# yuecideng/Misc3D

Hardware: AMD Instinct MI355X
Metric: RANSAC hypotheses/sec, 1M-pt cloud (inlier-score GB/s: roofline.algorithmic_reuse) (higher is better)
Workload: dtype f64 decisions (fp32 screen + fp64 recount)

## Files before the change

### include/misc3d_amd.h

```cpp
#ifndef MISC3D_AMD_H
#define MISC3D_AMD_H

#include <stddef.h>
#include <stdint.h>

#ifdef __cplusplus
extern "C" {
#endif

#define M3D_OK 1
#define M3D_FALSE 0
#define M3D_ERR_PROBABILITY (-1)
#define M3D_ERR_TOO_FEW_POINTS (-2)
#define M3D_ERR_NO_NORMALS (-3)
#define M3D_ERR_SIZE_MISMATCH (-4)
#define M3D_ERR_INVALID_ARG (-5)
#define M3D_ERR_DEVICE (-6)
#define M3D_ERR_INTERNAL (-7)
#define M3D_ERR_NON_FINITE (-8)

enum m3d_model_kind { M3D_PLANE = 0, M3D_SPHERE = 1, M3D_CYLINDER = 2 };

typedef struct m3d_stats {
    double fitness;
// ... 360 lines not shown
    uint64_t n_rays;
    uint64_t pair_tests;
    uint64_t nodes_visited;
} m3d_raycast_stats;
int m3d_raycast_pinhole(const m3d_raycast_mesh *meshes, size_t n_meshes, const double *poses, size_t n_poses, size_t n_frames,
                        int width, int height, double fx, double fy, double cx, double cy, int device, float *t_hit,
                        uint32_t *geometry_ids, uint32_t *primitive_ids, float *primitive_normals, m3d_raycast_stats *stats);

int m3d_match_mutual_nn(const double *feat_src, size_t n_src, const double *feat_dst, size_t n_dst,
                        int dim, int method, int n_trees, int device, size_t *out_src,
                        size_t *out_dst, size_t *k);
uint64_t m3d_match_last_fallbacks(void);

typedef struct m3d_comm m3d_comm;
#define M3D_COMM_ID_BYTES 128
int m3d_comm_unique_id(uint8_t id[M3D_COMM_ID_BYTES]);
m3d_comm *m3d_comm_create_rccl(const uint8_t id[M3D_COMM_ID_BYTES], int world, int rank, int device);
typedef int (*m3d_allgather_fn)(void *user, const void *send, void *recv, size_t bytes_per_rank);
m3d_comm *m3d_comm_create_host(int world, int rank, m3d_allgather_fn fn, void *user);
int m3d_comm_create_local(int world, m3d_comm **comms );
void m3d_comm_destroy(m3d_comm *comm);
int m3d_comm_world(const m3d_comm *comm);
int m3d_comm_rank(const m3d_comm *comm);
uint64_t m3d_comm_collectives(const m3d_comm *comm);

int m3d_cloud_fit_sharded(m3d_cloud *cloud, m3d_comm *comm, int kind, double threshold, size_t max_iteration,
                          double probability, const uint64_t *seed, double *params, size_t *inliers,
                          size_t *n_inliers, m3d_stats *stats);
int m3d_segment_plane_iterative_sharded(const double *xyz, size_t n, double threshold, int max_iteration,
                                        double min_ratio, const uint64_t *seed, int device, m3d_comm *comm,
                                        size_t max_clusters, double *planes, size_t *cluster_offsets,
                                        size_t *cluster_indices, size_t *n_clusters);
int m3d_segment_plane_iterative_multi(const double *xyz, size_t n, double threshold, int max_iteration,
                                      double min_ratio, const uint64_t *seed, const int *devices, int n_dev,
                                      size_t max_clusters, double *planes, size_t *cluster_offsets,
                                      size_t *cluster_indices, size_t *n_clusters);
int m3d_fit_multi(int kind, const double *xyz, const double *normals, size_t n, double threshold,
                  size_t max_iteration, double probability, const uint64_t *seed, const int *devices, int n_dev,
                  double *params, size_t *inliers, size_t *n_inliers, m3d_stats *stats);
int m3d_registration_ransac_sharded(const double *src, size_t n_src, const double *dst, size_t n_dst,
                                    const size_t *corr_src, const size_t *corr_dst, size_t m, double threshold,
                                    int max_iter, double edge_length_threshold, double confidence,
                                    const uint64_t *seed, int device, m3d_comm *comm, double T[16],
                                    m3d_reg_stats *stats);

typedef struct m3d_config {
    int32_t dense_scoring;
    int32_t speculative_refine;
    int32_t lead_hypotheses;
    int32_t score_groups_per_block;
    int32_t score_min_workgroups;
    int32_t dense_workgroups;
    int32_t reg_neighbour_lists;
    int32_t reg_prune;
    int32_t match_brute;
    int32_t match_fp32_screen;
    int32_t pool_limit_mb;
    int32_t kernel_timing;
    int32_t reg_sorted_lists;
    int32_t score_fp32_screen;
    int32_t cull_fp32;
    int32_t reg_fp32_screen;
    int32_t sorted_tombstones;
    int32_t score_mfma;
    int32_t score_mfma_groups;
    int32_t score_waves4;
    int32_t score_waves4_groups;
    int32_t score_phases;
    int32_t compact_one_pass;
    int32_t plane_bound;
    int32_t lanes;
    int32_t wait_spin_us;
    int32_t prestream;
    int32_t chunk_cap;
    int32_t first_chunk;
    int32_t reg_cells_per_radius;
    int32_t match_pipeline;
    int32_t reg_cache;
    int32_t device_aliases;
    int32_t lanes_eager;
    int32_t list_mask;
    int32_t mask_early;
    int32_t ref_bound;
} m3d_config;
void m3d_get_config(m3d_config *out);
int m3d_set_config(const m3d_config *in);

const char *m3d_last_error(void);
int m3d_device_count(void);
const char *m3d_version(void);

#ifdef __cplusplus
}
#endif
#endif
```

### include/misc3d_amd_bench.h

```cpp
#ifndef MISC3D_AMD_BENCH_H
#define MISC3D_AMD_BENCH_H

#include "misc3d_amd.h"

#ifdef __cplusplus
extern "C" {
#endif

int m3d_bench_time_score(m3d_cloud *cloud, int kind, double threshold, const uint32_t *samples,
                         size_t n_hypotheses, int reps, int mode, double *ms_avg,
                         uint64_t *listed_pairs);


int m3d_bench_fp64_issue_rate(int device, double ms_target, double *tera_lane_ops_per_s, double *ms_measured);

int m3d_bench_cloud_setup_ms(const m3d_cloud *cloud, double out[5]);

int m3d_bench_plane_upper_bounds(m3d_cloud *cloud, double threshold, const uint32_t *samples, size_t n_hypotheses,
                                 uint32_t *ub_out);
int m3d_bench_plane_ref_upper_bounds(m3d_cloud *cloud, double threshold, const uint32_t *samples, size_t n_hypotheses,
                                     size_t ref_index, uint32_t *ub_out);
int m3d_bench_upper_bounds(m3d_cloud *cloud, int kind, double threshold, const uint32_t *samples, size_t n_hypotheses,
                           uint32_t *ub_out);
int m3d_bench_last_segment_ms(double out[6]);

int m3d_bench_reg_checkers(const double *ps, const double *pd, const double *T, double edge_threshold,
                           double distance_threshold);

int m3d_bench_kabsch_sums(const double *src, const double *dst, size_t n, int device, double out[18]);

int m3d_bench_icp_sums(const double *src, size_t n_src, const double *dst, size_t n_dst, double max_correspondence_distance,
                       const double *T, int device, double out[29], int64_t *corr);

int m3d_bench_fps_force_path(int path);

int m3d_bench_knn_force_path(int path);

int m3d_bench_knn_tile_merge(const double *data, size_t n, int dim, const double *queries, size_t m, int kk, int pages,
                             int splits, uint32_t rows_per_split, int device, uint32_t *idx_out, uint64_t *d2_bits_out);

int m3d_bench_voxel_force_path(int path);

int m3d_bench_proximity_cutoffs(double dist, double angle_deg, double out[5]);

int m3d_bench_fpfh_pair_bins(const double *pairs, size_t m, int32_t *bins, double *features);

unsigned m3d_bench_match_last_path(void);

#ifdef __cplusplus
}
#endif
#endif
```

### misc3d_amd/capi.py

```python
from __future__ import annotations

import ctypes as C
import threading
import os
import sys
from dataclasses import dataclass

import numpy as np

_HERE = os.path.dirname(os.path.abspath(__file__))
FP_ORDER = int(os.environ.get("M3D_FP_ORDER", "0") or 0)
_VARIANT = os.environ.get("M3D_LIB_VARIANT", "")
LIB_PATH = os.path.join(_HERE, "lib", *([_VARIANT] if _VARIANT else ([f"order{FP_ORDER}"] if FP_ORDER else [])), "libmisc3d_amd.so")
HEADER_PATH = os.path.join(os.path.dirname(_HERE), "include", "misc3d_amd.h")

PLANE, SPHERE, CYLINDER = 0, 1, 2
MINIMAL_SAMPLE = {PLANE: 3, SPHERE: 4, CYLINDER: 2}
NUM_PARAMS = {PLANE: 4, SPHERE: 4, CYLINDER: 7}
MODEL_STRIDE = 8

OK, FALSE = 1, 0
ERR_PROBABILITY, ERR_TOO_FEW_POINTS, ERR_NO_NORMALS, ERR_SIZE_MISMATCH = -1, -2, -3, -4
ERR_INVALID_ARG, ERR_DEVICE, ERR_INTERNAL = -5, -6, -7
ERR_NON_FINITE = -8
# ... 152 lines not shown
        L.m3d_raycast_pinhole.argtypes = [C.c_void_p, C.c_size_t, C.c_void_p, C.c_size_t, C.c_size_t, C.c_int, C.c_int, C.c_double,
                                          C.c_double, C.c_double, C.c_double, C.c_int, C.c_void_p, C.c_void_p, C.c_void_p,
                                          C.c_void_p, C.c_void_p]
        L.m3d_proximity_segment.argtypes = [C.c_void_p, C.c_void_p, C.c_size_t, C.c_size_t, C.c_double, C.c_void_p,
                                            C.c_size_t, C.c_size_t, C.c_int, C.c_void_p, C.c_void_p, C.c_void_p, C.c_void_p,
                                            C.c_void_p]
        L.m3d_proximity_segment_nn.argtypes = [C.c_void_p, C.c_void_p, C.c_size_t, C.c_size_t, C.c_size_t, C.c_void_p,
                                               C.c_void_p, C.c_void_p, C.c_size_t, C.c_size_t, C.c_int, C.c_void_p,
                                               C.c_void_p, C.c_void_p, C.c_void_p, C.c_void_p]
        L.m3d_radius_neighbors.argtypes = [C.c_void_p, C.c_size_t, C.c_double, C.c_int, C.c_void_p, C.c_void_p, C.c_void_p,
                                           C.c_size_t, C.c_void_p]
        L.m3d_bench_proximity_cutoffs.argtypes = [C.c_double, C.c_double, C.c_void_p]
        L.m3d_knn_create.restype = C.c_void_p
        L.m3d_knn_create.argtypes = [C.c_void_p, C.c_size_t, C.c_int, C.c_int, C.c_void_p]
        L.m3d_knn_destroy.restype = None
        L.m3d_knn_destroy.argtypes = [C.c_void_p]
        L.m3d_knn_size.restype = C.c_size_t
        L.m3d_knn_size.argtypes = [C.c_void_p]
        L.m3d_knn_dim.argtypes = [C.c_void_p]
        L.m3d_knn_search.argtypes = [C.c_void_p, C.c_void_p, C.c_size_t, C.c_int, C.c_int64, C.c_double, C.c_size_t,
                                     C.c_void_p, C.c_void_p, C.c_void_p, C.c_void_p, C.c_void_p]
        L.m3d_bench_knn_force_path.argtypes = [C.c_int]
        L.m3d_bench_knn_tile_merge.argtypes = [C.c_void_p, C.c_size_t, C.c_int, C.c_void_p, C.c_size_t, C.c_int, C.c_int,
                                               C.c_int, C.c_uint32, C.c_int, C.c_void_p, C.c_void_p]
        L.m3d_estimate_normals.argtypes = [C.c_void_p, C.c_size_t, C.c_int, C.c_double, C.c_int, C.c_int, C.c_void_p, C.c_int,
                                           C.c_void_p, C.c_void_p]
        L.m3d_compute_fpfh.argtypes = [C.c_void_p, C.c_void_p, C.c_size_t, C.c_int, C.c_double, C.c_int, C.c_int, C.c_void_p,
                                       C.c_void_p]
        L.m3d_preprocess_fragment.argtypes = [C.c_void_p, C.c_void_p, C.c_size_t, C.c_double, C.c_int, C.c_void_p, C.c_void_p,
                                              C.c_void_p]
        L.m3d_bench_fpfh_pair_bins.argtypes = [C.c_void_p, C.c_size_t, C.c_void_p, C.c_void_p]
        L.m3d_match_last_fallbacks.restype = C.c_uint64
        L.m3d_match_last_fallbacks.argtypes = []
        L.m3d_match_mutual_nn.argtypes = [C.c_void_p, C.c_size_t, C.c_void_p, C.c_size_t, C.c_int, C.c_int, C.c_int,
                                          C.c_int, C.c_void_p, C.c_void_p, C.c_void_p]
        L.m3d_comm_unique_id.argtypes = [C.c_void_p]
        L.m3d_comm_create_rccl.restype = C.c_void_p
        L.m3d_comm_create_rccl.argtypes = [C.c_void_p, C.c_int, C.c_int, C.c_int]
        L.m3d_comm_create_host.restype = C.c_void_p
        L.m3d_comm_create_host.argtypes = [C.c_int, C.c_int, ALLGATHER_FN, C.c_void_p]
        L.m3d_comm_create_local.argtypes = [C.c_int, C.c_void_p]
        L.m3d_comm_destroy.restype = None
        L.m3d_comm_destroy.argtypes = [C.c_void_p]
        L.m3d_comm_world.argtypes = [C.c_void_p]
        L.m3d_comm_rank.argtypes = [C.c_void_p]
        L.m3d_comm_collectives.restype = C.c_uint64
        L.m3d_comm_collectives.argtypes = [C.c_void_p]
        L.m3d_cloud_fit_sharded.argtypes = [C.c_void_p, C.c_void_p, C.c_int, C.c_double, C.c_size_t, C.c_double, C.c_void_p,
                                            C.c_void_p, C.c_void_p, C.c_void_p, C.c_void_p]
        L.m3d_segment_plane_iterative_clouds.argtypes = [C.c_void_p, C.c_size_t, C.c_double, C.c_int, C.c_double,
                                                          C.c_void_p, C.c_int, C.c_size_t, C.c_void_p, C.c_void_p,
                                                          C.c_void_p, C.c_void_p, C.c_void_p]
        L.m3d_segment_plane_iterative_sharded.argtypes = [C.c_void_p, C.c_size_t, C.c_double, C.c_int, C.c_double,
                                                          C.c_void_p, C.c_int, C.c_void_p, C.c_size_t, C.c_void_p,
                                                          C.c_void_p, C.c_void_p, C.c_void_p]
        L.m3d_segment_plane_iterative_multi.argtypes = [C.c_void_p, C.c_size_t, C.c_double, C.c_int, C.c_double,
                                                        C.c_void_p, C.c_void_p, C.c_int, C.c_size_t, C.c_void_p,
                                                        C.c_void_p, C.c_void_p, C.c_void_p]
        L.m3d_fit_multi.argtypes = [C.c_int, C.c_void_p, C.c_void_p, C.c_size_t, C.c_double, C.c_size_t, C.c_double,
                                    C.c_void_p, C.c_void_p, C.c_int, C.c_void_p, C.c_void_p, C.c_void_p, C.c_void_p]
        L.m3d_registration_ransac_sharded.argtypes = [C.c_void_p, C.c_size_t, C.c_void_p, C.c_size_t, C.c_void_p,
                                                      C.c_void_p, C.c_size_t, C.c_double, C.c_int, C.c_double,
                                                      C.c_double, C.c_void_p, C.c_int, C.c_void_p, C.c_void_p,
                                                      C.c_void_p]
        L.m3d_bench_fp64_issue_rate.argtypes = [C.c_int, C.c_double, C.c_void_p, C.c_void_p]
        L.m3d_bench_cloud_setup_ms.argtypes = [C.c_void_p, C.c_void_p]
        L.m3d_bench_last_segment_ms.argtypes = [C.c_void_p]
        L.m3d_bench_reg_checkers.argtypes = [C.c_void_p, C.c_void_p, C.c_void_p, C.c_double, C.c_double]
        L.m3d_get_config.restype = None
        L.m3d_get_config.argtypes = [C.c_void_p]
        L.m3d_set_config.argtypes = [C.c_void_p]
        L.m3d_release_cached.restype = None
        L.m3d_release_cached.argtypes = [C.c_int]
        _lib = L
    return _lib


class Config(C.Structure):
    _fields_ = [(k, C.c_int32) for k in ("dense_scoring", "speculative_refine", "lead_hypotheses",
                                         "score_groups_per_block", "score_min_workgroups", "dense_workgroups",
                                         "reg_neighbour_lists", "reg_prune", "match_brute", "match_fp32_screen",
                                         "pool_limit_mb", "kernel_timing", "reg_sorted_lists", "score_fp32_screen",
                                         "cull_fp32", "reg_fp32_screen", "sorted_tombstones", "score_mfma", "score_mfma_groups", "score_waves4", "score_waves4_groups", "score_phases", "compact_one_pass", "plane_bound",
                                         "lanes", "wait_spin_us", "prestream", "chunk_cap", "first_chunk", "reg_cells_per_radius", "match_pipeline", "reg_cache", "device_aliases", "lanes_eager", "list_mask", "mask_early", "ref_bound")]


def fp64_issue_rate(device=0, ms_target=2.0):
    t, ms = C.c_double(0), C.c_double(0)
    _check(lib().m3d_bench_fp64_issue_rate(device, ms_target, C.cast(C.byref(t), C.c_void_p), C.cast(C.byref(ms), C.c_void_p)))
    return float(t.value), float(ms.value)


def match_last_path() -> int:
    f = lib().m3d_bench_match_last_path
    f.restype = C.c_uint
    f.argtypes = []
    return int(f())


def get_config() -> Config:
    c = Config()
    lib().m3d_get_config(C.byref(c))
    return c


def set_config(**kw) -> Config:
    old = get_config()
    new = get_config()
    for k, v in kw.items():
        if not hasattr(new, k):
            raise AttributeError(k)
        setattr(new, k, int(v))
    _check(lib().m3d_set_config(C.byref(new)))
    return old


def restore_config(cfg: Config):
    _check(lib().m3d_set_config(C.byref(cfg)))


class Comm:

    def __init__(self, handle, keep=None):
        if not handle:
            raise M3DError(ERR_DEVICE, last_error())
        self._h = handle
        self._keep = keep

    @classmethod
    def rccl(cls, group=None, device=0, world=None, rank=None):
        import torch
        import torch.distributed as dist
        if world is None:
            world, rank = (dist.get_world_size(group), dist.get_rank(group)) if dist.is_initialized() else (1, 0)
        ident = np.zeros(128, dtype=np.uint8)
        status = np.zeros(129, dtype=np.uint8)
        err = None
        if rank == 0:
            try:
                _check(lib().m3d_comm_unique_id(_p(ident)))
                status[:128] = ident
                status[128] = 1
            except M3DError as e:
                err = e
        if world > 1:
            t = torch.from_numpy(status)
            dist.broadcast(t, src=dist.get_global_rank(group, 0) if group is not None else 0, group=group)
        if not status[128]:
            raise err if err is not None else M3DError(-6, "rank 0 could not create an RCCL unique id")
        ident = np.ascontiguousarray(status[:128])
        libc = C.CDLL(None)
        sys.stdout.flush()
        libc.fflush(None)
        if os.environ.get("M3D_RCCL_KEEP_STDOUT") == "1":
            return cls(lib().m3d_comm_create_rccl(_p(ident), world, rank, device))
        saved = os.dup(1)
        os.dup2(2, 1)
        try:
            h = lib().m3d_comm_create_rccl(_p(ident), world, rank, device)
        finally:
            libc.fflush(None)
            os.dup2(saved, 1)
            os.close(saved)
        return cls(h)

    @classmethod
    def host(cls, world, rank, fn):
# ... 233 lines not shown
            self.close()
        except Exception:
            pass

    def __enter__(self):
        return self

    def __exit__(self, *a):
        self.close()

    def fit(self, kind, threshold=0.01, max_iteration=1000, probability=0.9999, seed=None,
            want_inliers=True, copy=True) -> Fit:
        params = np.zeros(NUM_PARAMS[kind])
        inl = None
        if want_inliers:
            inl = _seg_scratch(max(self.n_created, 1)) if copy else None
            if inl is None:
                inl = self._out_buf()
        ni = C.c_size_t(0)
        st = Stats()
        _s, sref = _seed_ref(seed)
        rc = _check(lib().m3d_cloud_fit(self._h, kind, threshold, max_iteration, probability, sref, _addr(params),
                                        _addr(inl), C.byref(ni), C.byref(st)))
        if want_inliers:
            inliers = inl[: ni.value].copy() if copy else inl[: ni.value]
        else:
            inliers = np.zeros(0, dtype=np.uint64)
        return Fit(rc, params, inliers, (st, ni.value))

    def fit_sharded(self, comm, kind, threshold=0.01, max_iteration=1000, probability=0.9999, seed=None,
                    want_inliers=True, copy=True) -> Fit:
        params = np.zeros(NUM_PARAMS[kind])
        inl = self._out_buf() if want_inliers else None
        ni = C.c_size_t(0)
        st = Stats()
        _s, sref = _seed_ref(seed)
        rc = _check(lib().m3d_cloud_fit_sharded(self._h, comm._h if comm is not None else None, kind, threshold,
                                                max_iteration, probability, sref, _addr(params), _addr(inl),
                                                C.byref(ni), C.byref(st)))
        if want_inliers:
            inliers = inl[: ni.value].copy() if copy else inl[: ni.value]
        else:
            inliers = np.zeros(0, dtype=np.uint64)
        return Fit(rc, params, inliers, (st, ni.value))

    def score_range(self, kind, threshold, samples, begin=0, end=None, want_models=True):
        samples = np.ascontiguousarray(samples, dtype=np.uint32).reshape(-1, MINIMAL_SAMPLE[kind])
        end = len(samples) if end is None else end
        cnt = np.empty(end - begin, dtype=np.uint32)
        val = np.empty(end - begin, dtype=np.uint8)
        mod = np.empty((end - begin, MODEL_STRIDE)) if want_models else None
        _check(lib().m3d_cloud_score_range(self._h, kind, threshold, _p(samples), begin, end, _p(cnt), _p(val),
                                           _p(mod)))
        return val, (mod[:, : NUM_PARAMS[kind]].copy() if want_models else None), cnt

    def time_score(self, kind, threshold, samples, reps=5, mode=0):
        samples = np.ascontiguousarray(samples, dtype=np.uint32).reshape(-1, MINIMAL_SAMPLE[kind])
        ms = C.c_double(0)
        listed = C.c_uint64(0)
        _check(lib().m3d_bench_time_score(self._h, kind, threshold, _p(samples), len(samples), reps, mode,
                                          C.cast(C.byref(ms), C.c_void_p), C.cast(C.byref(listed), C.c_void_p)))
        return float(ms.value), int(listed.value)

    def plane_upper_bounds(self, threshold, samples):
        samples = np.ascontiguousarray(samples, dtype=np.uint32).reshape(-1, 3)
        ub = np.zeros(len(samples), dtype=np.uint32)
        _check(lib().m3d_bench_plane_upper_bounds(self._h, threshold, _p(samples), len(samples), _p(ub)))
        return ub

    def plane_ref_upper_bounds(self, threshold, samples, ref_index):
        samples = np.ascontiguousarray(samples, dtype=np.uint32).reshape(-1, 3)
        ub = np.zeros(len(samples), dtype=np.uint32)
        f = lib().m3d_bench_plane_ref_upper_bounds
        f.argtypes = [C.c_void_p, C.c_double, C.c_void_p, C.c_size_t, C.c_size_t, C.c_void_p]
        _check(f(self._h, threshold, _p(samples), len(samples), int(ref_index), _p(ub)))
        return ub

    def upper_bounds(self, kind, threshold, samples):
        samples = np.ascontiguousarray(samples, dtype=np.uint32).reshape(-1, MINIMAL_SAMPLE[kind])
        ub = np.zeros(len(samples), dtype=np.uint32)
        _check(lib().m3d_bench_upper_bounds(self._h, kind, threshold, _p(samples), len(samples), _p(ub)))
        return ub

    def exact_error(self, kind, threshold, model):
        model = _f64(model)
        cnt = C.c_uint64(0)
        err = C.c_double(0)
        _check(lib().m3d_cloud_exact_error(self._h, kind, threshold, _p(model), C.cast(C.byref(cnt), C.c_void_p),
                                           C.cast(C.byref(err), C.c_void_p)))
        return int(cnt.value), float(err.value)

    refine_takes_expected = True

    def refine(self, kind, threshold, params, copy=True, expected=None):
        params = _f64(params).copy()
        inl = self._out_buf()
        ni = C.c_size_t(0)
        rc = _check(lib().m3d_cloud_refine_expect(self._h, kind, threshold, _p(params),
                                                  -1 if expected is None else int(expected), _p(inl),
                                                  C.cast(C.byref(ni), C.c_void_p)))
        return rc, params, (inl[: ni.value].copy() if copy else inl[: ni.value])

    def minimal_model(self, kind, threshold, sample_row):
        row = np.ascontiguousarray(sample_row, dtype=np.uint32).reshape(-1)
        if self.n == self.n_created:
            pts = np.ascontiguousarray(self._host_xyz[row])
            nrm = np.ascontiguousarray(self._host_nrm[row]) if self._host_nrm is not None else None
            model = np.zeros(8)
            ok = C.c_uint8(0)
            _check(lib().m3d_minimal_fit(kind, _p(pts), _p(nrm), _p(model), C.cast(C.byref(ok), C.c_void_p)))
            return model[: NUM_PARAMS[kind]].copy()
        _, mod, _ = self.score_range(kind, threshold, row.reshape(1, -1), 0, 1)
        return mod[0]

    def remove_inliers(self, kind, threshold, model):
        model = _f64(model).copy()
        nr = C.c_size_t(0)
        _check(lib().m3d_cloud_remove_inliers(self._h, kind, threshold, _p(model), C.cast(C.byref(nr), C.c_void_p)))
        self.n = int(lib().m3d_cloud_size(self._h))
        return nr.value


def draw_samples(n_points, kind, n_hyp, seed):
    out = np.zeros((n_hyp, MINIMAL_SAMPLE[kind]), dtype=np.uint32)
    _check(lib().m3d_draw_samples(n_points, kind, n_hyp, C.c_uint64(seed), _p(out)))
    return out


def fit(kind, xyz, normals=None, threshold=0.01, max_iteration=1000, probability=0.9999, seed=None,
        device=0, copy=True) -> Fit:
    xyz = _f64(xyz).reshape(-1, 3)
    n = len(xyz)
    params = np.zeros(NUM_PARAMS[kind])
    inl = _seg_scratch(max(n, 1))
    if inl is None:
        inl = np.empty(max(n, 1), dtype=np.uint64)
    ni = C.c_size_t(0)
    st = Stats()
    _s, sref = _seed_ref(seed)
    sp = C.cast(sref, C.c_void_p) if sref else None
    nip, stp = C.cast(C.byref(ni), C.c_void_p), C.cast(C.byref(st), C.c_void_p)
    if kind == CYLINDER:
        nrm = _f64(normals).reshape(-1, 3) if normals is not None else None
        rc = lib().m3d_fit_cylinder(_p(xyz), _p(nrm), n, threshold, max_iteration, probability, sp, device,
                                    _p(params), _p(inl), nip, stp)
    else:
        fn = lib().m3d_fit_plane if kind == PLANE else lib().m3d_fit_sphere
        rc = fn(_p(xyz), n, threshold, max_iteration, probability, sp, device, _p(params), _p(inl), nip, stp)
    _check(rc)
    d = st.asdict()
    d["n_inliers"] = int(ni.value)
    return Fit(rc, params, inl[: ni.value].copy() if copy else inl[: ni.value], d)


_seg_tls = threading.local()
_SEG_SCRATCH_MAX = 1 << 25


def _seg_scratch(n):
    if n > _SEG_SCRATCH_MAX:
        return None
    buf = getattr(_seg_tls, "buf", None)
    if buf is None or len(buf) < n:
        try:
            buf = np.asarray(_PinnedU64(n))
        except MemoryError:
# ... 940 lines not shown
```

### misc3d_amd/csrc/m3d_bound.hip

```cpp
#include "m3d_cull_kernels.hpp"

#include <cstdlib>

#include "m3d_bound_fp.hpp"
#include "m3d_config.hpp"
#include "m3d_eig3.hpp"
#include "m3d_fp.hpp"
#include "m3d_wave.hpp"

#pragma clang fp contract(off)

namespace m3d {

constexpr int kFrameLevels = 12;

__global__ __launch_bounds__(64) void tile_frames_k(const double* __restrict__ sx, const double* __restrict__ sy,
                                                     const double* __restrict__ sz, uint32_t n_tiles,
                                                     double* __restrict__ frames, uint16_t* __restrict__ cum) {
    __shared__ float pf[3][kTilePoints];
    __shared__ uint32_t hist[kBoundBins + 2];
    const int lane = threadIdx.x;
    const uint32_t tile = blockIdx.x;
    if (tile >= n_tiles) return;
    constexpr int P = kTilePoints / 64;
// ... 110 lines not shown
        if (!(m[0] >= 8.0)) break;
        const double in = 1.0 / m[0];
        const double mx = m[1] * in, my = m[2] * in, mz = m[3] * in;
        const double A[9] = {m[4] * in - mx * mx, m[5] * in - mx * my, m[6] * in - mx * mz,
                             m[5] * in - mx * my, m[7] * in - my * my, m[8] * in - my * mz,
                             m[6] * in - mx * mz, m[8] * in - my * mz, m[9] * in - mz * mz};
        double en[3];
        j3x3_smallest_eigvec(A, en);
        if (!((en[0] + en[1] + en[2]) * 0.0 == 0.0)) break;
        e[0] = en[0]; e[1] = en[1]; e[2] = en[2];
        c[0] += mx; c[1] += my; c[2] += mz;
        const double q = (e[0] * (A[0] * e[0] + A[1] * e[1] + A[2] * e[2]) + e[1] * (A[3] * e[0] + A[4] * e[1] + A[5] * e[2])) +
                         e[2] * (A[6] * e[0] + A[7] * e[1] + A[8] * e[2]);
        s = sqrt(fmax(q, 0.0));
        s = fmax(s, 1e-7 * ext);
        band = 3.5 * s;
    }
    const int kmin = (fabs(e[0]) <= fabs(e[1]) && fabs(e[0]) <= fabs(e[2])) ? 0 : (fabs(e[1]) <= fabs(e[2]) ? 1 : 2);
    const double a3[3] = {kmin == 0 ? 1.0 : 0.0, kmin == 1 ? 1.0 : 0.0, kmin == 2 ? 1.0 : 0.0};
    double u[3] = {e[1] * a3[2] - e[2] * a3[1], e[2] * a3[0] - e[0] * a3[2], e[0] * a3[1] - e[1] * a3[0]};
    const double ul = sqrt((u[0] * u[0] + u[1] * u[1]) + u[2] * u[2]);
    u[0] /= ul; u[1] /= ul; u[2] /= ul;
    const double v[3] = {e[1] * u[2] - e[2] * u[1], e[2] * u[0] - e[0] * u[2], e[0] * u[1] - e[1] * u[0]};
    const double wlo = -5.0 * s, invd = (double)kBoundBins / (10.0 * s);
    double U = 0.0, V = 0.0, W = 0.0, R = 0.0;
#pragma unroll
    for (int j = 0; j < P; ++j) {
        if (!fin[j]) continue;
        const double dx = px[j] - c[0], dy = py[j] - c[1], dz = pz[j] - c[2];
        const double w = (dx * e[0] + dy * e[1]) + dz * e[2];
        const double uu = (dx * u[0] + dy * u[1]) + dz * u[2];
        const double vv = (dx * v[0] + dy * v[1]) + dz * v[2];
        const double rx = ((dx - w * e[0]) - uu * u[0]) - vv * v[0];
        const double ry = ((dy - w * e[1]) - uu * u[1]) - vv * v[1];
        const double rz = ((dz - w * e[2]) - uu * u[2]) - vv * v[2];
        U = fmax(U, fabs(uu));
        V = fmax(V, fabs(vv));
        W = fmax(W, fabs(w));
        R = fmax(R, fmax(fabs(rx), fmax(fabs(ry), fabs(rz))));
        atomicAdd(&hist[bound_bin(w, wlo, invd)], 1u);
    }
    U = wave_max(U);
    V = wave_max(V);
    W = wave_max(W);
    R = wave_max(R);
    __syncthreads();
    {
        const uint32_t h0 = hist[2 * lane], h1 = hist[2 * lane + 1];
        const uint32_t own = h0 + h1, incl = wave_incl_scan(own, lane);
        const uint32_t excl = incl - own;
        cm[2 * lane] = (uint16_t)excl;
        cm[2 * lane + 1] = (uint16_t)(excl + h0);
        if (lane == 63) cm[kBoundBins + 2] = (uint16_t)incl;
    }
    const double Rm = R + 1e-13 * (mabs + ext);
    const bool ok = (U + V + W + Rm) < 1e12 && invd > 0.0 && invd < 1e30 && ext > 1e-12 && mabs < 1e12;
    if (lane == 0) {
        fr[0] = c[0]; fr[1] = c[1]; fr[2] = c[2];
        fr[3] = e[0]; fr[4] = e[1]; fr[5] = e[2];
        fr[6] = u[0]; fr[7] = u[1]; fr[8] = u[2];
        fr[9] = v[0]; fr[10] = v[1]; fr[11] = v[2];
        fr[12] = U; fr[13] = V; fr[14] = Rm; fr[15] = wlo; fr[16] = invd; fr[17] = W; fr[18] = nf;
        fr[19] = ok ? 1.0 : 0.0;
    }
}

void launch_tile_frames(const SortedView& s, double* frames, uint16_t* cum, hipStream_t st) {
    if (s.n_tiles) tile_frames_k<<<s.n_tiles, 64, 0, st>>>(s.x, s.y, s.z, s.n_tiles, frames, cum);
}

constexpr int kBoundWaves = 8;
template <int KIND , int kBoundTpw ,
          bool REF >
__global__ __launch_bounds__(64 * kBoundWaves, REF ? 6 : 1 ) void plane_bound_k(const double* __restrict__ frames, const uint16_t* __restrict__ cum,
                                                                   uint32_t n_tiles, double max_abs,
                                                                   const double* __restrict__ score,
                                                                   const unsigned long long* __restrict__ masks, uint32_t n_groups,
                                                                   const double* __restrict__ boxes, const float* __restrict__ cull32,
                                                                   uint32_t* __restrict__ surv_count,
                                                                   const uint32_t* __restrict__ surv,
                                                                   uint32_t* __restrict__ ubsum, const uint32_t* __restrict__ best_count,
                                                                   unsigned long long* __restrict__ keep,
                                                                   uint32_t* __restrict__ tickets ,
                                                                   uint32_t max_list, RefHistArgs ref, bool ref_alone) {
    constexpr int kBoundTpb = kBoundWaves * kBoundTpw;
    constexpr int kRefTpb = REF ? kBoundTpb : 1;
    static_assert(!REF || KIND == 0, "reference histograms bound planes");
    __shared__ double rt_s[kRefTpb][kRefTileStride];
    __shared__ __attribute__((aligned(8))) uint16_t rcm_s[kRefTpb][kRefCumStride];
    __shared__ float bx_s[kBoundTpb][6];
    __shared__ double c_s[kBoundTpb][3];
    __shared__ float f_s[kBoundTpb][kFrameStride];
    __shared__ __attribute__((aligned(8))) uint16_t cm_s[kBoundTpb][kCumStride];
    __shared__ uint32_t wsum[kBoundWaves][64];
    __shared__ double rec_s[64][9];
    __shared__ float q_s[64][13];
    const int lane = threadIdx.x & 63;
    const int wave = __builtin_amdgcn_readfirstlane((int)(threadIdx.x >> 6));
    const uint32_t total = surv_count[0];
    if (total > max_list) {
        if (blockIdx.x == 0 && blockIdx.y == 0 && threadIdx.x == 0) surv_count[0] = 0u;
        return;
    }
    if (blockIdx.x * 64u >= total) return;
    const uint32_t t0 = blockIdx.y * (uint32_t)kBoundTpb, nt = min((uint32_t)kBoundTpb, n_tiles - t0);
    double hv[6] = {0.0, 0.0, 0.0, 0.0, 0.0, 0.0};
    if (REF)
        for (int k = 0; k < 6; ++k) hv[k] = ref.hdr[k];
    const bool use_ref = REF && hv[0] != 0.0;
    RefPlane gp;
    gp.ok = false;
    if (REF) {
        gp = ref_plane_record(hv + 1, max_abs);
        const double* __restrict__ rsrc = ref.tiles + (size_t)t0 * kRefTileStride;
        for (uint32_t i = threadIdx.x; i < nt * (uint32_t)kRefTileStride; i += 64u * kBoundWaves) (&rt_s[0][0])[i] = rsrc[i];
        const uint32_t* __restrict__ csrc = reinterpret_cast<const uint32_t*>(ref.cum + (size_t)t0 * kRefCumStride);
        uint32_t* cdst = reinterpret_cast<uint32_t*>(&rcm_s[0][0]);
        for (uint32_t i = threadIdx.x; i < nt * (uint32_t)(kRefCumStride / 2); i += 64u * kBoundWaves) cdst[i] = csrc[i];
    }
    {
        const double* __restrict__ src = frames + (size_t)t0 * kFrameStride;
        for (uint32_t i = threadIdx.x; i < nt * (uint32_t)kFrameStride; i += 64u * kBoundWaves) {
            const uint32_t tl = i / (uint32_t)kFrameStride, k = i % (uint32_t)kFrameStride;
            const double v = src[i];
            if (k < 3u) c_s[tl][k] = v;
            f_s[tl][k] = frame_to_f32(v, k);
        }
        if (KIND != 0) {
            __syncthreads();
            if (threadIdx.x < nt) f_s[threadIdx.x][0] = cyl_tile_rho(f_s[threadIdx.x]);
        }
        if (cull32)
            for (uint32_t i = threadIdx.x; i < nt * 6u; i += 64u * kBoundWaves)
                bx_s[i / 6u][i % 6u] = reinterpret_cast<const float*>(boxes + (size_t)(t0 + i / 6u) * kBoxStride + 8)[i % 6u];
        const uint32_t* __restrict__ csrc = reinterpret_cast<const uint32_t*>(cum + (size_t)t0 * kCumStride);
        uint32_t* cdst = reinterpret_cast<uint32_t*>(&cm_s[0][0]);
        for (uint32_t i = threadIdx.x; i < nt * (uint32_t)(kCumStride / 2); i += 64u * kBoundWaves) cdst[i] = csrc[i];
    }
    for (uint32_t first = blockIdx.x * 64u; first < total; first += gridDim.x * 64u) {
        const uint32_t nb = min(64u, total - first);
        const bool has = (uint32_t)lane < nb;
        const uint32_t h = surv[first + (has ? (uint32_t)lane : 0u)];
        __syncthreads();
        {
            const uint32_t k = threadIdx.x & 7u;
#pragma unroll
            for (uint32_t si = threadIdx.x >> 3; si < 64u; si += (64u * kBoundWaves) >> 3) {
                const uint32_t hh = surv[first + min(si, nb - 1u)];
                rec_s[si][k] = score[(size_t)hh * kModelStride + k];
                if (cull32) {
                    q_s[si][k] = cull32[(size_t)(hh >> 1) * 24u + (hh & 1u) + 2u * k];
                    if (KIND == 2 && k < 3u) q_s[si][8u + k] = cull32[(size_t)(hh >> 1) * 24u + (hh & 1u) + 2u * (8u + k)];
                }
            }
        }
        __syncthreads();
        PlaneBoundRec pr;
        CylBoundRec cr;
        RefHypRec rr;
        if (KIND == 0) {
            pr = plane_bound_record(rec_s[lane], max_abs);
            pr.ok = pr.ok && has;
            if (REF && use_ref) rr = ref_hyp_record(gp, rec_s[lane], max_abs);
        } else {
            cr = KIND == 1 ? sphere_bound_record(rec_s[lane], max_abs) : cyl_bound_record(rec_s[lane], max_abs);
            cr.ok = cr.ok && has;
        }
        const unsigned long long bit = 1ull << (h & 63u);
        const unsigned long long* __restrict__ mrow = masks + (size_t)(h >> 6);
        bool tch[kBoundTpw];
        float q[11] = {0, 0, 0, 0, 0, 0, 0, 0, 0, 0, 0};
        if (cull32) {
#pragma unroll
            for (int k = 0; k < (KIND == 2 ? 11 : 8); ++k) q[k] = q_s[lane][k];
        } else {
#pragma unroll
            for (int i = 0; i < kBoundTpw; ++i) {
                const uint32_t tl = (uint32_t)(wave + kBoundWaves * i);
                tch[i] = (has && tl < nt) ? (mrow[(size_t)(t0 + tl) * n_groups] & bit) != 0ull : false;
            }
        }
        uint32_t ub = 0;
#pragma unroll
        for (int i = 0; i < kBoundTpw; ++i) {
            const int tl = wave + kBoundWaves * i;
            if (cull32 && KIND == 0) {
                const float* bx = bx_s[tl];
                const float sv = __builtin_fmaf(q[0], bx[0], __builtin_fmaf(q[1], bx[1], __builtin_fmaf(q[2], bx[2], q[3])));
                const float hx = __builtin_fmaxf(bx[3], 0.0f), hy = __builtin_fmaxf(bx[4], 0.0f), hz = __builtin_fmaxf(bx[5], 0.0f);
                const float rv = __builtin_fmaf(q[4], hx, __builtin_fmaf(q[5], hy, __builtin_fmaf(q[6], hz, q[7])));
                tch[i] = has && (uint32_t)tl < nt && bx[3] >= 0.0f && !(rv - __builtin_fabsf(sv) < 0.0f);
            } else if (cull32 && KIND == 2) {
                const float* bx = bx_s[tl];
                const bool live = bx[3] >= 0.0f;
                const float hx = live ? bx[3] : 0.0f, hy = live ? bx[4] : 0.0f, hz = live ? bx[5] : 0.0f;
                const float rb = __builtin_sqrtf(__builtin_fmaf(hz, hz, __builtin_fmaf(hy, hy, hx * hx))) * 1.000001f;
                const float d1 = __builtin_fmaf(q[0], bx[0], __builtin_fmaf(q[1], bx[1], __builtin_fmaf(q[2], bx[2], q[3])));
                const float d2 = __builtin_fmaf(q[4], bx[0], __builtin_fmaf(q[5], bx[1], __builtin_fmaf(q[6], bx[2], q[7])));
                const float tt = __builtin_fmaf(d2, d2, d1 * d1);
                const float dist = __builtin_sqrtf(tt);
                const float rt = q[8] * rb;
                const float t1 = (q[9] + rt) - dist;
                const float t2 = (dist + rt) - q[10];
                const float t = __uint_as_float(__float_as_uint(t1) | __float_as_uint(t2));
                tch[i] = has && (uint32_t)tl < nt && live && !(t < 0.0f);
            }
            if (__ballot(tch[i]) == 0ull) continue;
            uint32_t u_t = KIND == 0 ? plane_pair_ub(pr, c_s[tl], f_s[tl], cm_s[tl])
                                     : cyl_pair_ub(cr, c_s[tl], f_s[tl], f_s[tl][0], cm_s[tl]);
            if (REF && use_ref) {
                const uint32_t u_r = ref_pair_ub(rr, pr.a, pr.b, pr.c, pr.d, rt_s[tl], rcm_s[tl]);
                u_t = ref_alone ? u_r : min(u_t, u_r);
            }
            ub += tch[i] ? u_t : 0u;
        }
        wsum[wave][lane] = ub;
        __syncthreads();
        if (wave == 0) {
            uint32_t tot = 0;
#pragma unroll
            for (int w = 0; w < kBoundWaves; ++w) tot += wsum[w][lane];
            if (has && tot) atomicAdd(&ubsum[h], tot);
            __threadfence();
            const uint32_t blk = first / 64u;
            uint32_t old = 0;
            if (lane == 0) old = atomicAdd(&tickets[1u + blk], 1u);
            old = (uint32_t)__builtin_amdgcn_readfirstlane((int)old);
            if (old == gridDim.y - 1u) {
                __threadfence();
                const uint32_t best = best_count[0];
                const uint32_t sum = has ? atomicAdd(&ubsum[h], 0u) : 0u;
                if (has && best != 0u && sum < best) atomicAnd(&keep[h >> 6], ~bit);
                uint32_t done = 0;
                if (lane == 0) {
                    tickets[1u + blk] = 0u;
                    done = atomicAdd(&tickets[0], 1u);
                    if (done == (total + 63u) / 64u - 1u) {
                        tickets[0] = 0u;
                        surv_count[0] = 0u;
                    }
                }
            }
        }
    }
}

constexpr int kCylTpb = 64;
__global__ __launch_bounds__(64 * kBoundWaves) void cyl_bound_words_k(const double* __restrict__ frames, const uint16_t* __restrict__ cum,
                                                                       uint32_t n_tiles, double max_abs, const double* __restrict__ score,
                                                                       uint32_t* __restrict__ surv_count, const uint32_t* __restrict__ surv,
                                                                       uint32_t* __restrict__ ubsum, const uint32_t* __restrict__ best_count,
                                                                       unsigned long long* __restrict__ keep, uint32_t* __restrict__ tickets,
                                                                       uint32_t max_list, const unsigned long long* __restrict__ touched,
                                                                       uint32_t touched_stride) {
    __shared__ double c_s[kCylTpb][3];
    __shared__ float f_s[kCylTpb][kFrameStride];
    __shared__ __attribute__((aligned(8))) uint16_t cm_s[kCylTpb][kCumStride];
    const int lane = threadIdx.x & 63;
    const uint32_t wave = threadIdx.x >> 6;
    const uint32_t total = surv_count[0];
    if (total > max_list) {
        if (blockIdx.x == 0 && blockIdx.y == 0 && threadIdx.x == 0) surv_count[0] = 0u;
        return;
    }
    if (blockIdx.x * (64u * kBoundWaves) >= total) return;
    const uint32_t t0 = blockIdx.y * (uint32_t)kCylTpb, nt = min((uint32_t)kCylTpb, n_tiles - t0);
    {
        const double* __restrict__ src = frames + (size_t)t0 * kFrameStride;
        for (uint32_t i = threadIdx.x; i < nt * (uint32_t)kFrameStride; i += 64u * kBoundWaves) {
            const uint32_t tl = i / (uint32_t)kFrameStride, k = i % (uint32_t)kFrameStride;
            const double v = src[i];
            if (k < 3u) c_s[tl][k] = v;
            f_s[tl][k] = frame_to_f32(v, k);
        }
        __syncthreads();
        if (threadIdx.x < nt) f_s[threadIdx.x][0] = cyl_tile_rho(f_s[threadIdx.x]);
        const uint32_t* __restrict__ csrc = reinterpret_cast<const uint32_t*>(cum + (size_t)t0 * kCumStride);
        uint32_t* cdst = reinterpret_cast<uint32_t*>(&cm_s[0][0]);
        for (uint32_t i = threadIdx.x; i < nt * (uint32_t)(kCumStride / 2); i += 64u * kBoundWaves) cdst[i] = csrc[i];
        __syncthreads();
    }
    for (uint32_t first = (blockIdx.x * kBoundWaves + wave) * 64u; first < total; first += gridDim.x * (64u * kBoundWaves)) {
        const uint32_t nb = min(64u, total - first);
        const bool has = (uint32_t)lane < nb;
        const uint32_t h = surv[first + (has ? (uint32_t)lane : 0u)];
        double rec[8];
        {
            const double2* __restrict__ rp = reinterpret_cast<const double2*>(score + (size_t)h * kModelStride);
#pragma unroll
            for (int k = 0; k < 4; ++k) {
                const double2 v = rp[k];
                rec[2 * k] = v.x;
                rec[2 * k + 1] = v.y;
            }
        }
        CylBoundRec cr = cyl_bound_record(rec, max_abs);
        cr.ok = cr.ok && has;
        unsigned long long w0 = has ? touched[(size_t)(t0 / 64u) * touched_stride + h] : 0ull;
        unsigned long long w1 = (has && t0 + 64u < n_tiles) ? touched[(size_t)(t0 / 64u + 1u) * touched_stride + h] : 0ull;
        uint32_t ub = 0;
        for (uint32_t tl = 0; tl < nt; ++tl) {
            const bool mine = (((tl < 64u ? w0 : w1) >> (tl & 63u)) & 1ull) != 0ull;
            if (__builtin_amdgcn_ballot_w64(mine) == 0ull) continue;
            const uint32_t u_t = cyl_pair_ub(cr, c_s[tl], f_s[tl], f_s[tl][0], cm_s[tl]);
            ub += mine ? u_t : 0u;
        }
        if (has && ub) atomicAdd(&ubsum[h], ub);
        __threadfence();
        const uint32_t blk = first / 64u;
        uint32_t old = 0;
        if (lane == 0) old = atomicAdd(&tickets[1u + blk], 1u);
        old = (uint32_t)__builtin_amdgcn_readfirstlane((int)old);
        if (old == gridDim.y - 1u) {
            __threadfence();
            const uint32_t best = best_count[0];
            const uint32_t sum = has ? atomicAdd(&ubsum[h], 0u) : 0u;
            if (has && best != 0u && sum < best) atomicAnd(&keep[h >> 6], ~(1ull << (h & 63u)));
            if (lane == 0) {
                tickets[1u + blk] = 0u;
                const uint32_t done = atomicAdd(&tickets[0], 1u);
                if (done == (total + 63u) / 64u - 1u) {
                    tickets[0] = 0u;
                    surv_count[0] = 0u;
                }
            }
        }
    }
}

void launch_plane_bound(int kind, const SortedView& s, const double* score, const unsigned long long* masks, unsigned long long* keep,
                        uint32_t n_groups, uint32_t group_begin, uint32_t group_end, uint32_t* ubsum,
                        const uint32_t* best_count, uint32_t* surv_count, const uint32_t* surv, uint32_t* tickets,
                        const float* cull32, hipStream_t st, bool always, const unsigned long long* touched, uint32_t touched_stride,
                        const RefHistArgs* ref, bool ref_alone) {
    group_end = std::min(group_end, n_groups);
    if (!s.frames || !s.frame_cum || !s.n_tiles || !surv || !surv_count || !tickets || group_begin >= group_end) return;
    const uint32_t window = group_end - group_begin;
    constexpr uint32_t gdiv = 6;
    const uint32_t gx = std::min<uint32_t>(window, std::max<uint32_t>(4u, (window + gdiv - 1) / gdiv));
    constexpr int tpw = 8, tpw_cyl = 16;
    const uint32_t tpb = (uint32_t)(kBoundWaves * (kind == 0 ? tpw : tpw_cyl));
    const uint32_t max_list = always ? 0xFFFFFFFFu : window * 32u;
    if (kind == 2 && touched && s.radius < 1e18) {
        const dim3 gw((window + kBoundWaves - 1) / kBoundWaves, (s.n_tiles + kCylTpb - 1) / kCylTpb);
        cyl_bound_words_k<<<gw, 64 * kBoundWaves, 0, st>>>(s.frames, s.frame_cum, s.n_tiles, s.max_abs, score, surv_count, surv, ubsum, best_count,
                                                           keep, tickets, max_list, touched, touched_stride);
        return;
    }
    const dim3 g(gx, (s.n_tiles + tpb - 1) / tpb), b(64 * kBoundWaves);
    if (s.radius >= 1e18 || kind == 1) cull32 = nullptr;
    auto go = [&](auto kernel) {
        kernel<<<g, b, 0, st>>>(s.frames, s.frame_cum, s.n_tiles, s.max_abs, score, masks, n_groups, s.boxes, cull32, surv_count, surv,
                                ubsum, best_count, keep, tickets, max_list, (ref && kind == 0) ? *ref : RefHistArgs{}, ref_alone);
    };
    if (kind == 0 && ref) go(plane_bound_k<0, tpw, true>);
    else if (kind == 0) go(plane_bound_k<0, tpw, false>);
    else if (kind == 1) go(plane_bound_k<1, tpw_cyl, false>);
    else go(plane_bound_k<2, tpw_cyl, false>);
}

}
```

### misc3d_amd/csrc/m3d_config.cpp

```cpp
#include "m3d_config.hpp"

#include <algorithm>
#include <cstdlib>
#include <cstring>
#include <mutex>

#include "m3d_driver.hpp"

namespace m3d {
namespace {
m3d_config g_cfg;
std::once_flag g_once;
std::mutex g_cfg_mu;
thread_local m3d_config t_cfg;
thread_local int t_cfg_pins = 0;

long env_long(const char* name, long def) {
    const char* e = std::getenv(name);
    if (!e || !*e) return def;
    char* end = nullptr;
    const long v = std::strtol(e, &end, 10);
    return end == e ? def : v;
}
bool env_is(const char* name, char first) {
    const char* e = std::getenv(name);
    return e && e[0] == first;
}
void sanitize(m3d_config& c) {
    if (c.lead_hypotheses < 64 || c.lead_hypotheses % 64) c.lead_hypotheses = 128;
    if (c.score_groups_per_block < 1 || c.score_groups_per_block > 64) c.score_groups_per_block = 8;
    if (c.score_min_workgroups < 1) c.score_min_workgroups = 8192;
    if (c.dense_workgroups < 1) c.dense_workgroups = 8192;
    if (c.pool_limit_mb < 0) c.pool_limit_mb = 0;
    if (c.score_phases < -1 || c.score_phases == 1 || c.score_phases > 3) c.score_phases = -1;
    if (c.plane_bound < 0 || c.plane_bound > 2) c.plane_bound = 1;
    if (c.cull_fp32 < 0 || c.cull_fp32 > 2) c.cull_fp32 = 1;
    c.score_mfma = c.score_mfma_groups = c.score_waves4 = c.score_waves4_groups = c.compact_one_pass = 0;
    if (c.lanes < 1 || c.lanes > 8) c.lanes = 4;
    if (c.wait_spin_us < 0) c.wait_spin_us = 500;
    c.prestream = c.prestream != 0;
    c.chunk_cap = (int32_t)std::min<long>(std::max<long>(((long)c.chunk_cap + 63) / 64 * 64, 1024), 262144);
    c.first_chunk = c.first_chunk <= 0 ? 0 : (int32_t)std::min<long>(((long)c.first_chunk + 63) / 64 * 64, 1 << 20);
    if (c.reg_cells_per_radius < 1 || c.reg_cells_per_radius > 16) c.reg_cells_per_radius = 4;
    if (c.match_pipeline < 0 || c.match_pipeline > 2) c.match_pipeline = 1;
    if (c.reg_cache < 0 || c.reg_cache > 2) c.reg_cache = 1;
    if (c.device_aliases < 0) c.device_aliases = 0;
    if (c.device_aliases > 16) c.device_aliases = 16;
    if (c.lanes_eager < 1 || c.lanes_eager > 8) c.lanes_eager = 2;
    if (c.list_mask < 0) c.list_mask = 1;
    if (c.list_mask > 16) c.list_mask = 16;
    c.mask_early = c.mask_early != 0;
    if (c.ref_bound < 0 || c.ref_bound > 2) c.ref_bound = 1;
}
void load_env() {
    std::memset(&g_cfg, 0, sizeof(g_cfg));
    g_cfg.dense_scoring = env_is("M3D_DENSE", '1');
    g_cfg.speculative_refine = !env_is("M3D_SPEC", '0');
    g_cfg.lead_hypotheses = (int32_t)env_long("M3D_LEAD", 128);
    g_cfg.score_groups_per_block = (int32_t)env_long("M3D_GPB", 8);
    g_cfg.score_min_workgroups = (int32_t)env_long("M3D_SCORE_MIN_WGS", 8192);
    g_cfg.dense_workgroups = (int32_t)env_long("M3D_SCORE_WGS", 8192);
    g_cfg.reg_neighbour_lists = !env_is("M3D_REG_NL", '0');
    g_cfg.reg_prune = !env_is("M3D_REG_PRUNE", '0');
    g_cfg.match_brute = env_is("M3D_MATCH_BRUTE", '1');
    g_cfg.match_fp32_screen = env_is("M3D_MATCH_SCREEN", 'f');
    g_cfg.pool_limit_mb = (int32_t)env_long("M3D_POOL_MB", 4096);
    g_cfg.kernel_timing = env_is("M3D_KERNEL_TIMING", '1');
    g_cfg.reg_sorted_lists = !env_is("M3D_REG_SORTED", '0');
    g_cfg.score_fp32_screen = !env_is("M3D_SCORE_SCREEN", '0');
    g_cfg.cull_fp32 = env_is("M3D_CULL_FP32", '0') ? 0 : (env_is("M3D_CULL_FP32", '2') ? 2 : 1);
    g_cfg.reg_fp32_screen = !env_is("M3D_REG_SCREEN", '0');
    g_cfg.sorted_tombstones = !env_is("M3D_TOMBSTONES", '0');
    g_cfg.score_phases = (int32_t)env_long("M3D_SCORE_PHASES", -1);
    g_cfg.plane_bound = (int32_t)env_long("M3D_PLANE_BOUND", 1);
    g_cfg.lanes = (int32_t)env_long("M3D_LANES", 4);
    g_cfg.wait_spin_us = (int32_t)env_long("M3D_SPIN_US", 500);
    g_cfg.prestream = !env_is("M3D_PRESTREAM", '0');
    g_cfg.chunk_cap = (int32_t)env_long("M3D_CHUNK_CAP", 24576);
    g_cfg.first_chunk = (int32_t)env_long("M3D_FIRST_CHUNK", 2048);
    g_cfg.reg_cells_per_radius = (int32_t)env_long("M3D_REG_K", 4);
    g_cfg.match_pipeline = (int32_t)env_long("M3D_MATCH_PIPELINE", 1);
    g_cfg.reg_cache = (int32_t)env_long("M3D_REG_CACHE", 1);
    g_cfg.device_aliases = (int32_t)env_long("M3D_DEVICE_ALIASES", 0);
    g_cfg.lanes_eager = (int32_t)env_long("M3D_LANES_EAGER", 2);
    g_cfg.list_mask = (int32_t)env_long("M3D_LIST_MASK", 1);
    g_cfg.mask_early = !env_is("M3D_MASK_EARLY", '0');
    g_cfg.ref_bound = (int32_t)env_long("M3D_REF_BOUND", 1);
    sanitize(g_cfg);
}
}

const m3d_config& config() {
    std::call_once(g_once, load_env);
    if (t_cfg_pins > 0) return t_cfg;
    std::lock_guard<std::mutex> lock(g_cfg_mu);
    t_cfg = g_cfg;
    return t_cfg;
}
void config_pin() {
    std::call_once(g_once, load_env);
    if (t_cfg_pins++ == 0) {
        std::lock_guard<std::mutex> lock(g_cfg_mu);
        t_cfg = g_cfg;
    }
}
void config_unpin() {
    if (t_cfg_pins > 0) --t_cfg_pins;
}
void config_store(const m3d_config& c) {
    std::call_once(g_once, load_env);
    m3d_config n = c;
    sanitize(n);
    std::lock_guard<std::mutex> lock(g_cfg_mu);
    g_cfg = n;
}
}

extern "C" {
void m3d_get_config(m3d_config* out) {
    if (out) *out = m3d::config();
}
int m3d_set_config(const m3d_config* in) {
    if (!in) return m3d::fail(M3D_ERR_INVALID_ARG, "invalid argument");
    if (in->score_mfma || in->score_waves4 || in->compact_one_pass)
        return m3d::fail(M3D_ERR_INVALID_ARG, "score_mfma / score_waves4 / compact_one_pass: retired, must be 0 (the variants were removed)");
    m3d::config_store(*in);
    return M3D_OK;
}
}
```

### misc3d_amd/csrc/m3d_cull_kernels.hip

```cpp
#include "m3d_cull_kernels.hpp"
#include "m3d_poison.hpp"

#include <hip/hip_ext.h>

#include <cstdlib>
#include <type_traits>

#include "m3d_config.hpp"
#include "m3d_fp.hpp"
#include "m3d_ref_hist.hpp"
#include "m3d_tile_count.hpp"
#include "m3d_wave.hpp"

#pragma clang fp contract(off)

namespace m3d {

typedef float f32x2 __attribute__((ext_vector_type(2)));

__global__ __launch_bounds__(256) void tile_boxes_k(const double* __restrict__ sx, const double* __restrict__ sy,
                                                     const double* __restrict__ sz, uint32_t n_tiles,
                                                     double* __restrict__ boxes, double ox, double oy, double oz,
                                                     float* __restrict__ tile_f32) {
    const int lane = threadIdx.x & 63;
// ... 634 lines not shown
    return std::min<uint32_t>(window >= 192u ? 2u * g : (thinned ? g + g / 2u : g), kScreenMaxGroups);
}
constexpr int kCntStride = 64;

template <int KIND, int Q>
__device__ __forceinline__ void screen_eval(const float4 ra, const float4 rb, const float4 rc, const f32x2 (&xf)[Q],
                                            const f32x2 (&yf)[Q], const f32x2 (&zf)[Q], const f32x2 (&wf)[Q] ,
                                            uint32_t& bits, float& m) {
    uint32_t acc = 0;
    float mn = __builtin_inff();
    if (KIND == 0) {
        const f32x2 A = {ra.x, ra.x}, B = {ra.y, ra.y}, C = {ra.z, ra.z}, D = {rb.x, rb.x}, M2 = {-ra.w, -ra.w};
        f32x2 s[Q];
#pragma unroll
        for (int j = 0; j < Q; ++j) s[j] = __builtin_elementwise_fma(C, zf[j], D);
#pragma unroll
        for (int j = 0; j < Q; ++j) s[j] = __builtin_elementwise_fma(B, yf[j], s[j]);
#pragma unroll
        for (int j = 0; j < Q; ++j) s[j] = __builtin_elementwise_fma(A, xf[j], s[j]);
#pragma unroll
        for (int j = 0; j < Q; ++j) s[j] = __builtin_elementwise_fma(s[j], s[j], M2);
#pragma unroll
        for (int j = 0; j < Q; ++j) {
            acc = __builtin_amdgcn_alignbit(acc, __float_as_uint(s[j].x), 31);
            acc = __builtin_amdgcn_alignbit(acc, __float_as_uint(s[j].y), 31);
            mn = __builtin_fminf(__builtin_fminf(mn, __builtin_fabsf(s[j].x)), __builtin_fabsf(s[j].y));
        }
    } else if (KIND == 2) {
        const f32x2 AX = {ra.x, ra.x}, AY = {ra.y, ra.y}, AZ = {ra.z, ra.z}, AD = {ra.w, ra.w};
        const f32x2 BX = {rb.x, rb.x}, BY = {rb.y, rb.y}, BZ = {rb.z, rb.z}, BD = {rb.w, rb.w};
        const f32x2 MID = {-rc.x, -rc.x}, H2 = {-rc.y, -rc.y};
        f32x2 d1[Q], d2[Q];
#pragma unroll
        for (int j = 0; j < Q; ++j) {
            d1[j] = __builtin_elementwise_fma(AZ, zf[j], AD);
            d2[j] = __builtin_elementwise_fma(BZ, zf[j], BD);
        }
#pragma unroll
        for (int j = 0; j < Q; ++j) {
            d1[j] = __builtin_elementwise_fma(AY, yf[j], d1[j]);
            d2[j] = __builtin_elementwise_fma(BY, yf[j], d2[j]);
        }
#pragma unroll
        for (int j = 0; j < Q; ++j) {
            d1[j] = __builtin_elementwise_fma(AX, xf[j], d1[j]);
            d2[j] = __builtin_elementwise_fma(BX, xf[j], d2[j]);
        }
#pragma unroll
        for (int j = 0; j < Q; ++j) d1[j] = __builtin_elementwise_fma(d1[j], d1[j], MID);
#pragma unroll
        for (int j = 0; j < Q; ++j) d1[j] = __builtin_elementwise_fma(d2[j], d2[j], d1[j]);
#pragma unroll
        for (int j = 0; j < Q; ++j) d1[j] = __builtin_elementwise_fma(d1[j], d1[j], H2);
#pragma unroll
        for (int j = 0; j < Q; ++j) {
            acc = __builtin_amdgcn_alignbit(acc, __float_as_uint(d1[j].x), 31);
            acc = __builtin_amdgcn_alignbit(acc, __float_as_uint(d1[j].y), 31);
            mn = __builtin_fminf(__builtin_fminf(mn, __builtin_fabsf(d1[j].x)), __builtin_fabsf(d1[j].y));
        }
    } else {
        const f32x2 CX = {rb.x, rb.x}, CY = {rb.y, rb.y}, CZ = {rb.z, rb.z}, KK = {ra.x, ra.x}, H2 = {-ra.y, -ra.y};
        f32x2 t[Q];
#pragma unroll
        for (int j = 0; j < Q; ++j) t[j] = wf[j] + KK;
#pragma unroll
        for (int j = 0; j < Q; ++j) t[j] = __builtin_elementwise_fma(CX, xf[j], t[j]);
#pragma unroll
        for (int j = 0; j < Q; ++j) t[j] = __builtin_elementwise_fma(CY, yf[j], t[j]);
#pragma unroll
        for (int j = 0; j < Q; ++j) t[j] = __builtin_elementwise_fma(CZ, zf[j], t[j]);
#pragma unroll
        for (int j = 0; j < Q; ++j) t[j] = __builtin_elementwise_fma(t[j], t[j], H2);
#pragma unroll
        for (int j = 0; j < Q; ++j) {
            acc = __builtin_amdgcn_alignbit(acc, __float_as_uint(t[j].x), 31);
            acc = __builtin_amdgcn_alignbit(acc, __float_as_uint(t[j].y), 31);
            mn = __builtin_fminf(__builtin_fminf(mn, __builtin_fabsf(t[j].x)), __builtin_fabsf(t[j].y));
        }
    }
    bits = acc;
    m = mn;
}

template <int KIND, bool OWN_BOX_TESTS>
__device__ __forceinline__ void score_screen_body(const double* __restrict__ sx, const double* __restrict__ sy,
                                                  const double* __restrict__ sz,
                                                  const double* __restrict__ boxes, double max_abs,
                                                  const double* __restrict__ score,
                                                  unsigned long long* __restrict__ masks,
                                                  const unsigned long long* __restrict__ keep,
                                                  uint32_t n_groups, uint32_t groups_per_block ,
                                                  uint32_t* __restrict__ counts_rep, uint32_t rep_stride,
                                                  uint32_t* __restrict__ pair_rep,
                                                  uint32_t group_begin, uint32_t group_end, uint32_t block_x, uint32_t block_y,
                                                  const float* __restrict__ cull32, const float* __restrict__ tile_f32,
                                                  uint32_t has_dead ) {
    __shared__ uint16_t ids[kScreenMaxGroups * 64];
    __shared__ __attribute__((aligned(16))) uint8_t cnt8[64 * kCntStride];
    constexpr int NL = KIND == 2 ? 3 : 2;
    __shared__ float4 loc[64 + 1][NL];
    const int lane = threadIdx.x & 63;
    const uint32_t tile = block_x;
    uint32_t* __restrict__ counts = counts_rep + (size_t)(tile % kCountReplicas) * rep_stride;
    const uint32_t g0 = group_begin + block_y * groups_per_block;
    unsigned long long mm = 0;
    if (OWN_BOX_TESTS) {
        const float* __restrict__ f = reinterpret_cast<const float*>(boxes + (size_t)tile * kBoxStride + 8);
        const float bx = f[0], by = f[1], bz = f[2];
        float hx = f[3], hy = f[4], hz = f[5];
        const bool live = hx >= 0.0f;
        if (!live) hx = hy = hz = 0.0f;
        const float rb = __builtin_sqrtf(__builtin_fmaf(hz, hz, __builtin_fmaf(hy, hy, hx * hx))) * 1.000001f;
        for (uint32_t w = 0; w < groups_per_block && g0 + w < group_end; ++w) {
            const uint32_t h = (g0 + w) * 64u + (uint32_t)lane;
            const float t = cull32_one<KIND>(cull32 + (size_t)(h >> 1) * 24u, (int)(h & 1u), bx, by, bz, hx, hy, hz, rb);
            const unsigned long long word = live ? __ballot(!(t < 0.0f)) : 0ull;
            if (lane == 0) masks[(size_t)tile * n_groups + g0 + w] = word;
            if ((uint32_t)lane == w) mm = word & keep[g0 + w];
        }
    } else if ((uint32_t)lane < groups_per_block && g0 + lane < group_end) {
        mm = masks[(size_t)tile * n_groups + g0 + lane] & keep[g0 + lane];
    }
    if (!__ballot(mm != 0)) return;
    const size_t base = (size_t)tile * kTilePoints + lane;
    constexpr int P = kTilePoints / 64, Q = P / 2;
    double box[6];
#pragma unroll
    for (int k = 0; k < 6; ++k) box[k] = boxes[(size_t)tile * kBoxStride + k];
    f32x2 xf[Q], yf[Q], zf[Q];
    bool tile_screened;
    if (tile_f32) {
        const f32x2* __restrict__ t2 = reinterpret_cast<const f32x2*>(tile_f32 + (size_t)tile * kTileF32Floats) + lane;
#pragma unroll
        for (int j = 0; j < Q; ++j) {
            xf[j] = t2[(0 * Q + j) * 64];
            yf[j] = t2[(1 * Q + j) * 64];
            zf[j] = t2[(2 * Q + j) * 64];
        }
        tile_screened = boxes[(size_t)tile * kBoxStride + 6] != 0.0;
    } else {
        float chk = 0.0f;
#pragma unroll
        for (int j = 0; j < Q; ++j) {
            xf[j] = {(float)(sx[base + 128 * j] - box[0]), (float)(sx[base + 128 * j + 64] - box[0])};
            yf[j] = {(float)(sy[base + 128 * j] - box[1]), (float)(sy[base + 128 * j + 64] - box[1])};
            zf[j] = {(float)(sz[base + 128 * j] - box[2]), (float)(sz[base + 128 * j + 64] - box[2])};
            chk += ((xf[j].x + xf[j].y) + (yf[j].x + yf[j].y)) + (zf[j].x + zf[j].y);
        }
        tile_screened = __ballot(!(chk * 0.0f == 0.0f)) == 0ull;
    }
    f32x2 wf[Q];
    if (KIND == 1) {
#pragma unroll
        for (int j = 0; j < Q; ++j) {
            f32x2 w = xf[j] * xf[j];
            w = __builtin_elementwise_fma(yf[j], yf[j], w);
            wf[j] = __builtin_elementwise_fma(zf[j], zf[j], w);
        }
    }
    uint32_t dead8 = 0;
    bool tile_has_dead = false;
    if (KIND == 0 && has_dead && tile_f32) {
#pragma unroll
        for (int j = 0; j < Q; ++j) dead8 = (dead8 << 2) | (xf[j].x != xf[j].x ? 2u : 0u) | (xf[j].y != xf[j].y ? 1u : 0u);
        tile_has_dead = tile_screened && __ballot(dead8 != 0u) != 0ull;
    }
    uint32_t total = 0;
    const int mm_lo = (int)(uint32_t)mm, mm_hi = (int)(uint32_t)(mm >> 32);
    for (uint32_t w = 0; w < groups_per_block; ++w) {
        const uint32_t lo = (uint32_t)__builtin_amdgcn_readlane(mm_lo, (int)w), hi = (uint32_t)__builtin_amdgcn_readlane(mm_hi, (int)w);
        if ((lo | hi) == 0u) continue;
        const unsigned long long word = ((unsigned long long)hi << 32) | lo;
        const uint32_t slot = __builtin_amdgcn_mbcnt_hi(hi, __builtin_amdgcn_mbcnt_lo(lo, total));
        if (__builtin_amdgcn_inverse_ballot_w64(word)) ids[slot] = (uint16_t)(w * 64u + (uint32_t)lane);
        total += (uint32_t)__popcll(word);
    }
    __syncthreads();
    if (threadIdx.x == 0) atomicAdd(&pair_rep[(tile + block_y * 67u) % (uint32_t)kPairMain], total);
    const double* __restrict__ score0 = score + (size_t)g0 * 64u * kModelStride;
    auto exact_count = [&](uint32_t id) -> uint32_t {
        double rec[kModelStride];
        const double* __restrict__ rp = score0 + (size_t)id * kModelStride;
#pragma unroll
        for (int k = 0; k < kModelStride; ++k) rec[k] = rp[k];
        uint32_t c = 0;
#pragma unroll 1
        for (int half = 0; half < 2; ++half) {
            double x[P / 2], y[P / 2], z[P / 2];
#pragma unroll
            for (int j = 0; j < P / 2; ++j) {
                x[j] = sx[base + 64 * (half * (P / 2) + j)];
                y[j] = sy[base + 64 * (half * (P / 2) + j)];
                z[j] = sz[base + 64 * (half * (P / 2) + j)];
            }
            c += tile_count<KIND, P / 2>(rec, x, y, z);
        }
        return c;
    };
    for (uint32_t b0 = 0; b0 < total; b0 += 64u) {
        const uint32_t nb = min(64u, total - b0);
        const int my = (b0 + (uint32_t)lane < total) ? (int)ids[b0 + lane] : 0;
        {
            const double* __restrict__ rp = score0 + (size_t)my * kModelStride;
            constexpr int kRec = KIND == 2 ? 8 : 5;
            double rec[kRec];
#pragma unroll
            for (int k = 0; k < kRec; ++k) rec[k] = rp[k];
            float sr[12];
            if (KIND == 0) plane_screen_record(rec, box, max_abs, sr);
            else if (KIND == 1) sphere_screen_record(rec, box, max_abs, sr);
            else cylinder_screen_record(rec, box, max_abs, sr);
            loc[lane][0] = make_float4(sr[0], sr[1], sr[2], sr[3]);
            loc[lane][1] = make_float4(sr[4], sr[5], sr[6], sr[7]);
            if (KIND == 2) loc[lane][NL - 1] = make_float4(sr[8], sr[9], sr[10], sr[11]);
        }
        __syncthreads();
        uint32_t park = 0;
        auto step = [&](auto screened, auto dead, const float4 ra, const float4 rb, const float4 rc, uint32_t k, uint8_t* cnt_row) {
            constexpr bool SCREENED = decltype(screened)::value;
            constexpr bool DEAD = decltype(dead)::value;
            uint32_t bits = 0;
            bool exact = true;
            if (SCREENED) {
                float m;
                screen_eval<KIND, Q>(ra, rb, rc, xf, yf, zf, wf, bits, m);
                if (DEAD) bits &= ~dead8;
                exact = __ballot(!(m >= (KIND == 0 ? rb.y : (KIND == 1 ? rb.w : rc.z)))) != 0ull;
            }
            if (__builtin_expect(exact, 0)) {
                const uint32_t e = exact_count((uint32_t)__builtin_amdgcn_readlane(my, (int)k));
                if (lane == 0) atomicAdd(&pair_rep[(uint32_t)kPairMain + tile % (uint32_t)(kPairLead - kPairMain)], 1u);
                park = ((uint32_t)lane == k) ? e : park;
                bits = 0;
            }
            *cnt_row = (uint8_t)bits;
        };
        auto batch = [&](auto screened, auto dead) {
            uint32_t rec_off = 0, cnt_off = (uint32_t)lane;
            asm volatile("" : "+v"(rec_off), "+v"(cnt_off));
            const char* const loc_b = reinterpret_cast<const char*>(&loc[0][0]);
            auto fetch = [&](int i, float4& r0, float4& r1, float4& r2) {
                const float4* __restrict__ r = reinterpret_cast<const float4*>(loc_b + rec_off) + i * NL;
                r0 = r[0];
                r1 = r[1];
                r2 = r[NL - 1];
                __builtin_amdgcn_sched_barrier(0);
            };
            float4 a0, a1, a2, b0r, b1r, b2r;
            fetch(0, a0, a1, a2);
            for (uint32_t k = 0; k < nb; k += 4u) {
                fetch(1, b0r, b1r, b2r);
                step(screened, dead, a0, a1, a2, k, cnt8 + cnt_off);
                fetch(2, a0, a1, a2);
                if (k + 1u < nb) step(screened, dead, b0r, b1r, b2r, k + 1u, cnt8 + cnt_off + kCntStride);
                fetch(3, b0r, b1r, b2r);
                if (k + 2u < nb) step(screened, dead, a0, a1, a2, k + 2u, cnt8 + cnt_off + 2 * kCntStride);
                fetch(4, a0, a1, a2);
                if (k + 3u < nb) step(screened, dead, b0r, b1r, b2r, k + 3u, cnt8 + cnt_off + 3 * kCntStride);
                rec_off += 4u * NL * (uint32_t)sizeof(float4);
                cnt_off += 4u * kCntStride;
            }
        };
        if (tile_screened && !tile_has_dead) batch(std::true_type{}, std::false_type{});
        else if (tile_screened) batch(std::true_type{}, std::true_type{});
        else batch(std::false_type{}, std::false_type{});
        __syncthreads();
        if ((uint32_t)lane < nb) {
            const uint4* row = reinterpret_cast<const uint4*>(cnt8 + (uint32_t)lane * kCntStride);
            uint32_t sum = park;
#pragma unroll
            for (int i = 0; i < 4; ++i) {
                const uint4 v = row[i];
                sum += (uint32_t)__popc(v.x);
                sum += (uint32_t)__popc(v.y);
                sum += (uint32_t)__popc(v.z);
                sum += (uint32_t)__popc(v.w);
            }
            if (sum) atomicAdd(&counts[g0 * 64u + (uint32_t)my], sum);
        }
        __syncthreads();
    }
}
__device__ __forceinline__ uint32_t phase_tile4(uint32_t bx, uint32_t res_mask) {
    const uint32_t k = (uint32_t)__popc(res_mask);
    uint32_t m = res_mask;
    for (uint32_t j = bx % k; j > 0; --j) m &= m - 1u;
    return (bx / k) * 4u + (uint32_t)(__ffs(m) - 1);
}
template <int KIND>
__global__ __launch_bounds__(64) void score_screen_k(const double* __restrict__ sx, const double* __restrict__ sy,
                                                      const double* __restrict__ sz,
                                                      const double* __restrict__ boxes, double max_abs,
                                                      const double* __restrict__ score,
                                                      const unsigned long long* __restrict__ masks,
                                                      const unsigned long long* __restrict__ keep,
                                                      uint32_t n_groups, uint32_t groups_per_block ,
                                                      uint32_t* __restrict__ counts_rep, uint32_t rep_stride,
                                                      uint32_t* __restrict__ pair_rep,
                                                      uint32_t group_begin, uint32_t group_end,
                                                      const float* __restrict__ tile_f32, uint32_t has_dead,
                                                      uint32_t n_tiles, uint32_t res_mask) {
    uint32_t tile = blockIdx.x;
    if (res_mask != 0xFu) tile = phase_tile4(blockIdx.x, res_mask);
    if (tile >= n_tiles) return;
    score_screen_body<KIND, false>(sx, sy, sz, boxes, max_abs, score, const_cast<unsigned long long*>(masks), keep, n_groups,
                                   groups_per_block, counts_rep, rep_stride, pair_rep, group_begin, group_end, tile,
                                   blockIdx.y, nullptr, tile_f32, has_dead);
}

__global__ __launch_bounds__(64) void phase_keep_k(const uint32_t* __restrict__ counts_rep, uint32_t rep_stride,
                                                    const uint32_t* __restrict__ ub, const uint32_t* __restrict__ ubp,
                                                    const uint32_t* __restrict__ best_count_ptr,
                                                    unsigned long long* __restrict__ keep, uint32_t group_offset, uint32_t done_mask) {
    const uint32_t g = group_offset + blockIdx.x;
    const uint32_t h = g * 64u + threadIdx.x;
    const unsigned long long kw = keep[g];
    if (kw == 0ull) return;
    const uint32_t best = best_count_ptr[0];
    uint32_t c = 0;
#pragma unroll
    for (int r = 0; r < kCountReplicas; ++r) c += counts_rep[(size_t)r * rep_stride + h];
    const uint32_t ab = ubp[h];
    uint32_t done = 0;
    if (done_mask & 1u) done += ab & 0xFFFFu;
    if (done_mask & 2u) done += ab >> 16;
    const uint32_t rem = ub[h] - done;
    const bool k = ((kw >> threadIdx.x) & 1ull) && (best == 0u || (uint64_t)c + (uint64_t)rem * kTilePoints >= best);
    const unsigned long long m = __ballot(k);
    if (threadIdx.x == 0) keep[g] = m;
}

template <int KIND>
__global__ __launch_bounds__(64) void cull_lead_k(const double* __restrict__ sx, const double* __restrict__ sy,
                                                   const double* __restrict__ sz, const double* __restrict__ boxes,
                                                   uint32_t n_tiles, double max_abs, const double* __restrict__ score,
                                                   const float* __restrict__ cull32, unsigned long long* __restrict__ masks,
                                                   const unsigned long long* __restrict__ keep, uint32_t n_groups,
                                                   uint32_t lead_groups, uint32_t lead_gpb, uint32_t n_lead_wgs,
                                                   uint32_t* __restrict__ counts_rep, uint32_t rep_stride,
                                                   uint32_t* __restrict__ pair_rep, uint32_t* __restrict__ ub,
                                                   uint32_t cull_begin, uint32_t cull_end, uint32_t cull_gpw, uint32_t cull_tblocks,
                                                   const float* __restrict__ tile_f32, uint32_t has_dead, uint32_t* __restrict__ ubp) {
    if (blockIdx.x < n_lead_wgs) {
        score_screen_body<KIND, true>(sx, sy, sz, boxes, max_abs, score, masks, keep, n_groups, lead_gpb, counts_rep, rep_stride,
                                      pair_rep, 0u, lead_groups, blockIdx.x % n_tiles, blockIdx.x / n_tiles, cull32, tile_f32, has_dead);
    } else {
        const uint32_t b = blockIdx.x - n_lead_wgs;
        cull32_body<KIND>(boxes, n_tiles, cull32, n_groups, cull_gpw, masks, ub, cull_begin, cull_end, b % cull_tblocks,
                          b / cull_tblocks, ubp);
    }
}

__global__ void sum_replicas_k(const uint32_t* __restrict__ counts_rep, uint32_t rep_stride, uint32_t h_end,
                               uint32_t* __restrict__ counts, const uint32_t* __restrict__ pair_rep,
                               uint32_t* __restrict__ pairs_out, const uint8_t* __restrict__ valid, uint32_t h_count,
                               uint32_t* __restrict__ best_count, uint32_t h_begin,
                               uint32_t* __restrict__ counts_dev , PickFinal pf,
                               const unsigned long long* __restrict__ keep_final ) {
    const uint32_t h = h_begin + blockIdx.x * 256u + threadIdx.x;
    if (blockIdx.x == 0 && pair_rep && pairs_out) {
        __shared__ uint32_t red[256];
        uint32_t p = 0;
        for (int r = threadIdx.x; r < kPairMain; r += 256) p += pair_rep[r];
        red[threadIdx.x] = p;
        __syncthreads();
        for (int w = 128; w > 0; w >>= 1) {
            if ((int)threadIdx.x < w) red[threadIdx.x] += red[threadIdx.x + w];
            __syncthreads();
        }
        if (threadIdx.x == 0) {
            uint32_t e = 0;
            for (int r = kPairMain; r < kPairLead; ++r) e += pair_rep[r];
            pairs_out[0] = red[0];
            pairs_out[1] = e;
            pairs_out[2] = pair_rep[kPairLead];
        }
    }
    const bool mine = h < h_end;
    uint32_t c = 0;
    if (mine) {
#pragma unroll
        for (int r = 0; r < kCountReplicas; ++r) c += counts_rep[(size_t)r * rep_stride + h];
        if (keep_final && !((keep_final[h >> 6] >> (h & 63u)) & 1ull)) c = 0u;
    }
    const bool ok = mine && valid && h < h_count && valid[h];
    if (mine) {
        const uint32_t rec = valid ? (c | (ok ? 0x80000000u : 0u)) : c;
        if (counts) counts[h] = rec;
        if (counts_dev) counts_dev[h] = rec;
    }
    if (best_count) {
        uint32_t v = ok ? c : 0u;
        v = wave_max(v);
        if ((threadIdx.x & 63) == 0 && v) atomicMax(best_count, v);
    }
    if (!pf.pick) return;
    __shared__ uint32_t s_last, s_take, s_idx, s_tie;
    {
        unsigned long long key = (ok && c) ? (((unsigned long long)c << 32) | (0xFFFFFFFFu - h)) : 0ull;
        key = wave_max(key);
        if ((threadIdx.x & 63) == 0 && key) atomicMax(pf.key, key);
        if (pf.key2) {
            unsigned long long key2 = (ok && c) ? (((unsigned long long)c << 32) | h) : 0ull;
            key2 = wave_max(key2);
            if ((threadIdx.x & 63) == 0 && key2) atomicMax(pf.key2, key2);
        }
    }
    asm volatile("s_waitcnt vmcnt(0)" ::: "memory");
    __syncthreads();
    if (threadIdx.x == 0) {
        __threadfence_system();
        s_last = __hip_atomic_fetch_add(pf.ticket, 1u, __ATOMIC_RELAXED, __HIP_MEMORY_SCOPE_AGENT) == gridDim.x - 1 ? 1u : 0u;
    }
    __syncthreads();
    if (!s_last) return;
    if (threadIdx.x == 0) {
        const unsigned long long key = __hip_atomic_load(pf.key, __ATOMIC_RELAXED, __HIP_MEMORY_SCOPE_AGENT);
        const uint32_t cnt = (uint32_t)(key >> 32), idx = 0xFFFFFFFFu - (uint32_t)key;
        BestPick* pick = pf.pick;
        const bool had = !pf.first_chunk && pick->have;
        const bool take = cnt > 0 && (!had || cnt > pick->cnt);
        uint32_t tie = (pf.first_chunk || !had) ? 0u : pick->tie;
        if (pf.key2) {
            const unsigned long long k2 = __hip_atomic_load(pf.key2, __ATOMIC_RELAXED, __HIP_MEMORY_SCOPE_AGENT);
            const bool inner = cnt > 0 && (uint32_t)k2 != idx;
            if (take) tie = inner ? 1u : 0u;
            else if (had && cnt > 0 && cnt == pick->cnt) tie = 1u;
            *pf.key2 = 0ull;
        }
        s_take = take ? 1u : 0u;
        s_idx = idx;
        s_tie = tie;
        if (take) {
            pick->have = 1;
            pick->cnt = cnt;
            pick->index = pf.index_base + idx;
        } else if (!had) {
            pick->have = 0;
            pick->cnt = 0;
            pick->index = ~0ull;
        }
        pick->tie = tie;
        pf.pick_host->have = pick->have;
        pf.pick_host->cnt = pick->cnt;
        pf.pick_host->index = pick->index;
        pf.pick_host->tie = tie;
        *pf.key = 0ull;
        *pf.ticket = 0u;
    }
    __syncthreads();
    if (threadIdx.x < kModelStride) {
        if (s_take) pf.pick->params[threadIdx.x] = pf.params[(size_t)s_idx * kModelStride + threadIdx.x];
        else if (pf.first_chunk) pf.pick->params[threadIdx.x] = 0.0;
        if (s_tie && threadIdx.x == 0) pf.pick->params[0] = __builtin_nan("");
    }
    __syncthreads();
    if (threadIdx.x == 0) {
        __threadfence_system();
        __hip_atomic_store(&pf.pick_host->seq, pf.seq, __ATOMIC_RELEASE, __HIP_MEMORY_SCOPE_SYSTEM);
    }
}
void launch_sum_replicas(const uint32_t* counts_rep, uint32_t rep_stride, uint32_t h_end, uint32_t* counts,
                         const uint32_t* pair_rep, uint32_t* pairs_out, const uint8_t* valid, uint32_t h_count,
                         uint32_t* best_count, hipStream_t st, uint32_t h_begin, uint32_t* counts_dev, const PickFinal* pick,
                         const unsigned long long* keep_final) {
    PickFinal pf;
    if (pick) pf = *pick;
    if (h_end > h_begin)
        sum_replicas_k<<<(h_end - h_begin + 255) / 256, 256, 0, st>>>(counts_rep, rep_stride, h_end, counts, pair_rep,
                                                                      pairs_out, valid, h_count, best_count, h_begin,
                                                                      counts_dev, pf, keep_final);
}

bool launch_cull_lead(int kind, const SortedView& s, const double* score, const float* cull32, unsigned long long* masks,
                      const unsigned long long* keep, uint32_t n_groups, uint32_t lead_groups, uint32_t* counts_rep,
                      uint32_t rep_stride, uint32_t* pair_rep, uint32_t* ub, uint32_t cull_end, hipStream_t st, uint32_t* ubp) {
    cull_end = std::min(cull_end, n_groups);
    if (!s.n_tiles || !cull32 || !(s.radius < 1e18) || config().cull_fp32 == 0 || config().score_fp32_screen == 0 ||
        lead_groups == 0 || lead_groups > (uint32_t)kScreenMaxGroups || lead_groups >= cull_end)
        return false;
    const uint32_t lead_gpb = lead_groups;
    const uint32_t lead_y = 1;
    const uint32_t n_lead_wgs = s.n_tiles * lead_y;
    const uint32_t window = cull_end - lead_groups;
    const uint32_t tblocks = (s.n_tiles + 63) / 64;
    uint32_t gpw = std::max<uint32_t>(1, (uint32_t)(((uint64_t)tblocks * window) / 8192));
    gpw = std::min<uint32_t>(gpw, 8);
    const uint32_t cull_y = (window + gpw - 1) / gpw;
    const dim3 g(n_lead_wgs + tblocks * cull_y), b(64);
    if (kind == 0)
        cull_lead_k<0><<<g, b, 0, st>>>(s.x, s.y, s.z, s.boxes, s.n_tiles, s.max_abs, score, cull32, masks, keep, n_groups, lead_groups,
                                        lead_gpb, n_lead_wgs, counts_rep, rep_stride, pair_rep, ub, lead_groups, cull_end, gpw, tblocks,
                                        (const float*)s.tile_f32, s.has_dead ? 1u : 0u, ubp);
    else if (kind == 1)
        cull_lead_k<1><<<g, b, 0, st>>>(s.x, s.y, s.z, s.boxes, s.n_tiles, s.max_abs, score, cull32, masks, keep, n_groups, lead_groups,
                                        lead_gpb, n_lead_wgs, counts_rep, rep_stride, pair_rep, ub, lead_groups, cull_end, gpw, tblocks,
                                        (const float*)s.tile_f32, s.has_dead ? 1u : 0u, ubp);
    else
        cull_lead_k<2><<<g, b, 0, st>>>(s.x, s.y, s.z, s.boxes, s.n_tiles, s.max_abs, score, cull32, masks, keep, n_groups, lead_groups,
                                        lead_gpb, n_lead_wgs, counts_rep, rep_stride, pair_rep, ub, lead_groups, cull_end, gpw, tblocks,
                                        (const float*)s.tile_f32, s.has_dead ? 1u : 0u, ubp);
    return true;
}

__global__ __launch_bounds__(1024) void pick_best_k(const uint32_t* __restrict__ records, uint32_t count,
                                                     unsigned long long index_base, const double* __restrict__ params,
                                                     int first_chunk, BestPick* __restrict__ pick,
                                                     BestPickHost* __restrict__ pick_host,
                                                     uint32_t* __restrict__ records_host, uint32_t* __restrict__ best_count) {
    __shared__ uint32_t s_cnt[1024];
    __shared__ uint32_t s_idx[1024];
    __shared__ int s_take;
    uint32_t bc = 0, bi = 0xFFFFFFFFu;
    for (uint32_t i = threadIdx.x; i < count; i += 1024u) {
        const uint32_t r = records[i];
        if (records_host) records_host[i] = r;
        const uint32_t c = r & 0x7FFFFFFFu;
        if ((r >> 31) && c > bc) {
            bc = c;
            bi = i;
        }
    }
    s_cnt[threadIdx.x] = bc;
    s_idx[threadIdx.x] = bi;
    __syncthreads();
    for (int off = 512; off > 0; off >>= 1) {
        if ((int)threadIdx.x < off) {
            const uint32_t c2 = s_cnt[threadIdx.x + off], i2 = s_idx[threadIdx.x + off];
            const uint32_t c1 = s_cnt[threadIdx.x], i1 = s_idx[threadIdx.x];
            if (c2 > c1 || (c2 == c1 && i2 < i1)) {
                s_cnt[threadIdx.x] = c2;
                s_idx[threadIdx.x] = i2;
            }
        }
        __syncthreads();
    }
    if (threadIdx.x == 0) {
        if (best_count && s_cnt[0]) atomicMax(best_count, s_cnt[0]);
        const bool had = !first_chunk && pick->have;
        const bool take = s_cnt[0] > 0 && (!had || s_cnt[0] > pick->cnt);
        s_take = take ? 1 : 0;
        if (take) {
            pick->have = 1;
            pick->cnt = s_cnt[0];
            pick->index = index_base + s_idx[0];
        } else if (!had) {
            pick->have = 0;
            pick->cnt = 0;
            pick->index = ~0ull;
        }
        pick_host->have = pick->have;
        pick_host->cnt = pick->cnt;
        pick_host->index = pick->index;
        pick->tie = 0;
        pick_host->tie = 0;
    }
    __syncthreads();
    if (threadIdx.x < kModelStride) {
        if (s_take) pick->params[threadIdx.x] = params[(size_t)s_idx[0] * kModelStride + threadIdx.x];
        else if (first_chunk) pick->params[threadIdx.x] = 0.0;
    }
}
void launch_pick_best(const uint32_t* records, uint32_t count, unsigned long long index_base, const double* params,
                      bool first_chunk, BestPick* pick, BestPickHost* pick_host, hipStream_t st, uint32_t* records_host,
                      uint32_t* best_count) {
    pick_best_k<<<1, 1024, 0, st>>>(records, count, index_base, params, first_chunk ? 1 : 0, pick, pick_host,
                                    records_host, best_count);
}

void launch_score_mask(int kind, const SortedView& s, const double* score, const unsigned long long* masks,
                       const unsigned long long* keep, uint32_t n_groups, uint32_t* counts_rep, uint32_t rep_stride,
                       uint32_t* pair_rep, hipStream_t st, uint32_t group_begin, uint32_t group_end, hipEvent_t ev_start,
                       hipEvent_t ev_stop, bool thinned) {
    group_end = std::min(group_end, n_groups);
    if (!s.n_tiles || group_begin >= group_end) return;
    const uint32_t window = group_end - group_begin;
    const bool screened = config().score_fp32_screen != 0;
    const uint32_t gpb_max = screened ? screen_gpb_max(window, thinned) : std::min<uint32_t>((uint32_t)config().score_groups_per_block, 64u);
    const uint32_t min_wgs = (uint32_t)config().score_min_workgroups;
    const uint32_t gpb = std::max<uint32_t>(1, std::min<uint32_t>(gpb_max, (uint32_t)(((uint64_t)s.n_tiles * window) / min_wgs)));
    const dim3 g(screened ? (s.n_tiles + 7u) / 8u * 8u : s.n_tiles, (window + gpb - 1) / gpb), b(64);
    auto go = [&](auto kernel, auto... args) {
        if (ev_start && ev_stop) hipExtLaunchKernelGGL(kernel, g, b, 0, st, ev_start, ev_stop, 0, args...);
        else kernel<<<g, b, 0, st>>>(args...);
    };
    if (screened) {
        if (kind == 0)
            go(score_screen_k<0>, s.x, s.y, s.z, s.boxes, s.max_abs, score, masks, keep, n_groups, gpb, counts_rep, rep_stride, pair_rep,
               group_begin, group_end, (const float*)s.tile_f32, s.has_dead ? 1u : 0u, s.n_tiles, 0xFu);
        else if (kind == 1)
            go(score_screen_k<1>, s.x, s.y, s.z, s.boxes, s.max_abs, score, masks, keep, n_groups, gpb, counts_rep, rep_stride, pair_rep,
               group_begin, group_end, (const float*)s.tile_f32, s.has_dead ? 1u : 0u, s.n_tiles, 0xFu);
        else
            go(score_screen_k<2>, s.x, s.y, s.z, s.boxes, s.max_abs, score, masks, keep, n_groups, gpb, counts_rep, rep_stride, pair_rep,
               group_begin, group_end, (const float*)s.tile_f32, s.has_dead ? 1u : 0u, s.n_tiles, 0xFu);
    } else {
        if (kind == 0)
            go(score_mask_k<0>, s.x, s.y, s.z, score, masks, keep, n_groups, gpb, counts_rep, rep_stride, pair_rep, group_begin, group_end);
        else if (kind == 1)
            go(score_mask_k<1>, s.x, s.y, s.z, score, masks, keep, n_groups, gpb, counts_rep, rep_stride, pair_rep, group_begin, group_end);
        else
            go(score_mask_k<2>, s.x, s.y, s.z, score, masks, keep, n_groups, gpb, counts_rep, rep_stride, pair_rep, group_begin, group_end);
    }
}


int score_phases_for(int kind) {
    const int c = config().score_phases;
    if (c == 2 || c == 3) return c;
    return (c < 0 && kind == 2) ? 3 : 0;
}
bool launch_score_phased(int kind, const SortedView& s, const double* score, const unsigned long long* masks,
                         unsigned long long* keep, uint32_t n_groups, uint32_t* counts_rep, uint32_t rep_stride,
                         uint32_t* pair_rep, const uint32_t* ub, const uint32_t* ubp, const uint32_t* best_count, hipStream_t st,
                         uint32_t group_begin, uint32_t group_end, hipEvent_t ev_start, hipEvent_t ev_stop) {
    group_end = std::min(group_end, n_groups);
    const bool forced = config().score_phases >= 2;
    if (!ub || !ubp || !best_count || !s.tile_f32 || s.n_tiles < (forced ? 8u : 256u) || s.n_tiles > 200000u || score_phases_for(kind) == 0 ||
        config().score_fp32_screen == 0 || group_begin >= group_end || group_end - group_begin < (forced ? 2u : 32u))
        return false;
    const uint32_t window = group_end - group_begin;
    const uint32_t gpb_max = screen_gpb_max(window);
    const uint32_t min_wgs = (uint32_t)config().score_min_workgroups;
    const int n_ph = score_phases_for(kind);
    const uint32_t res[3] = {0x1u, n_ph == 3 ? 0x2u : 0xEu, 0xCu};
    uint32_t done = 0;
    for (int ph = 0; ph < n_ph; ++ph) {
        const uint32_t k = (uint32_t)__builtin_popcount(res[ph]);
        const uint32_t tiles_x = (s.n_tiles + 3u) / 4u * k;
        const uint32_t gpb = std::max<uint32_t>(1, std::min<uint32_t>(gpb_max, (uint32_t)(((uint64_t)tiles_x * window) / min_wgs)));
        const dim3 g((tiles_x + 7u) / 8u * 8u, (window + gpb - 1) / gpb), b(64);
        hipEvent_t e0 = ph == 0 ? ev_start : nullptr, e1 = ph == n_ph - 1 ? ev_stop : nullptr;
        auto go = [&](auto kernel) {
            if (ev_start && ev_stop && (e0 || e1))
                hipExtLaunchKernelGGL(kernel, g, b, 0, st, e0, e1, 0, s.x, s.y, s.z, s.boxes, s.max_abs, score, masks,
                                      (const unsigned long long*)keep, n_groups, gpb, counts_rep, rep_stride, pair_rep, group_begin, group_end,
                                      (const float*)s.tile_f32, s.has_dead ? 1u : 0u, s.n_tiles, res[ph]);
            else
                kernel<<<g, b, 0, st>>>(s.x, s.y, s.z, s.boxes, s.max_abs, score, masks, (const unsigned long long*)keep, n_groups, gpb, counts_rep,
                                        rep_stride, pair_rep, group_begin, group_end, (const float*)s.tile_f32, s.has_dead ? 1u : 0u, s.n_tiles, res[ph]);
        };
        if (kind == 0) go(score_screen_k<0>);
        else if (kind == 1) go(score_screen_k<1>);
        else go(score_screen_k<2>);
        done |= res[ph];
        if (ph + 1 < n_ph) phase_keep_k<<<window, 64, 0, st>>>(counts_rep, rep_stride, ub, ubp, best_count, keep, group_begin, done);
    }
    return true;
}

__global__ void count_bits_k(const unsigned long long* __restrict__ masks, const unsigned long long* __restrict__ keep,
                             uint32_t n_tiles, uint32_t n_groups, unsigned long long* __restrict__ total) {
    const size_t i = (size_t)blockIdx.x * 256u + threadIdx.x;
    unsigned long long c = 0;
    if (i < (size_t)n_tiles * n_groups) c = (unsigned long long)__popcll(masks[i] & keep[i % n_groups]);
    c = wave_sum(c);
    if ((threadIdx.x & 63) == 0 && c) atomicAdd(total, c);
}
void launch_count_bits(const unsigned long long* masks, const unsigned long long* keep, uint32_t n_tiles,
// ... 8 lines not shown
```

### misc3d_amd/csrc/m3d_cull_kernels.hpp

```cpp
#pragma once
#include "m3d_bound_fp.hpp"
#include "m3d_kernels.hpp"

namespace m3d {

constexpr int kTilePoints = 512;
constexpr int kBoxStride = 12;
constexpr int kCull32Stride = 12;
constexpr uint32_t kGroupsPerBlock = 8;

struct SortedView {
    const double* x;
    const double* y;
    const double* z;
    const double* boxes;
    uint32_t n_tiles;
    float* tile_f32 = nullptr;
    const double* frames = nullptr;
    const uint16_t* frame_cum = nullptr;
    bool has_dead = false;
    double max_abs = __builtin_inf();
    double origin[3] = {0.0, 0.0, 0.0};
    double radius = __builtin_inf();
};

constexpr int kTileF32Floats = 3 * kTilePoints;
void launch_tile_frames(const SortedView& s, double* frames, uint16_t* cum, hipStream_t st);
struct RefHistArgs {
    const double* sx = nullptr;
    const double* sy = nullptr;
    const double* sz = nullptr;
    uint32_t n_tiles = 0;
    const double* score = nullptr;
    const uint32_t* counts_rep = nullptr;
    uint32_t rep_stride = 0, lead = 0;
    const uint8_t* valid = nullptr;
    uint32_t h_count = 0, fixed_index = 0;
    uint32_t min_count = 1;
    double max_abs = 0.0;
    double* hdr = nullptr;
    double* tiles = nullptr;
    uint16_t* cum = nullptr;
};
inline size_t ref_hist_bytes(uint32_t n_tiles) {
    return sizeof(double) * (kRefHdrDoubles + (size_t)kRefTileStride * n_tiles) + sizeof(uint16_t) * (size_t)kRefCumStride * n_tiles;
}
inline void ref_hist_place(RefHistArgs& a, void* block) {
    a.hdr = static_cast<double*>(block);
    a.tiles = a.hdr + kRefHdrDoubles;
    a.cum = reinterpret_cast<uint16_t*>(a.tiles + (size_t)kRefTileStride * a.n_tiles);
}
void launch_ref_hist(const RefHistArgs& a, hipStream_t st);
void launch_plane_bound(int kind, const SortedView& s, const double* score, const unsigned long long* masks, unsigned long long* keep,
                        uint32_t n_groups, uint32_t group_begin, uint32_t group_end, uint32_t* ubsum,
                        const uint32_t* best_count, uint32_t* surv_count, const uint32_t* surv, uint32_t* tickets,
                        const float* cull32, hipStream_t st,
                        bool always = false ,
                        const unsigned long long* touched = nullptr ,
                        uint32_t touched_stride = 0,
                        const RefHistArgs* ref = nullptr ,
                        bool ref_alone = false );
void launch_tile_boxes(const SortedView& s, double* boxes, hipStream_t st);
PoisonJob make_poison_job(const SortedView& s, const double* model, double thr, uint32_t* total);
void launch_poison_plane_inliers(const PoisonJob& job, hipStream_t st);


void launch_cull_mask(int kind, const SortedView& s, const double* score, const uint8_t* valid, uint32_t h_count,
                      uint32_t n_groups, unsigned long long* masks, uint32_t* ub, hipStream_t st,
                      bool ub_is_zero = false, uint32_t group_begin = 0,
                      uint32_t group_end = 0xFFFFFFFFu ,
                      const float* cull32 = nullptr ,
                      uint32_t* ubp = nullptr ,
                      unsigned long long* touched = nullptr ,
                      uint32_t touched_stride = 0, bool* touched_written = nullptr );
void launch_keep_mask(const uint32_t* ub, const uint32_t* best_count, uint32_t n_groups, unsigned long long* keep,
                      hipStream_t st, uint32_t* zero_counts_rep = nullptr, uint32_t rep_stride = 0,
                      uint32_t group_offset = 0 ,
                      uint32_t* surv_count = nullptr, uint32_t* surv = nullptr );
constexpr int kCountReplicas = 16;
constexpr int kPairReplicas = 1024;
constexpr int kPairLead = kPairReplicas - 1;
constexpr int kPairMain = 1008;
void launch_score_mask(int kind, const SortedView& s, const double* score, const unsigned long long* masks,
                       const unsigned long long* keep, uint32_t n_groups, uint32_t* counts_rep, uint32_t rep_stride,
                       uint32_t* pair_rep ,
                       hipStream_t st, uint32_t group_begin = 0, uint32_t group_end = 0xFFFFFFFFu ,
                       hipEvent_t ev_start = nullptr, hipEvent_t ev_stop = nullptr ,
                       bool thinned = false );
bool launch_cull_lead(int kind, const SortedView& s, const double* score, const float* cull32, unsigned long long* masks,
                      const unsigned long long* keep, uint32_t n_groups, uint32_t lead_groups, uint32_t* counts_rep,
                      uint32_t rep_stride, uint32_t* pair_rep, uint32_t* ub, uint32_t cull_end, hipStream_t st, uint32_t* ubp = nullptr);
int score_phases_for(int kind);
bool launch_score_phased(int kind, const SortedView& s, const double* score, const unsigned long long* masks,
                         unsigned long long* keep, uint32_t n_groups, uint32_t* counts_rep, uint32_t rep_stride,
                         uint32_t* pair_rep, const uint32_t* ub, const uint32_t* ubp, const uint32_t* best_count, hipStream_t st,
                         uint32_t group_begin, uint32_t group_end, hipEvent_t ev_start, hipEvent_t ev_stop);
struct BestPick {
    unsigned long long index;
    uint32_t cnt, have;
    double params[8];
    uint32_t tie, pad;
};
struct BestPickHost {
    unsigned long long index;
    uint32_t cnt, have;
    uint32_t seq, tie;
};
struct PickFinal {
    unsigned long long* key = nullptr;
    unsigned long long* key2 = nullptr;
    uint32_t* ticket = nullptr;
    const double* params = nullptr;
    unsigned long long index_base = 0;
    int first_chunk = 0;
    BestPick* pick = nullptr;
    BestPickHost* pick_host = nullptr;
    uint32_t seq = 0;
};
void launch_sum_replicas(const uint32_t* counts_rep, uint32_t rep_stride, uint32_t h_end, uint32_t* counts,
                         const uint32_t* pair_rep, uint32_t* pairs_out, const uint8_t* valid, uint32_t h_count,
                         uint32_t* best_count, hipStream_t st, uint32_t h_begin = 0 ,
                         uint32_t* counts_dev = nullptr ,
                         const PickFinal* pick = nullptr,
                         const unsigned long long* keep_final = nullptr );
void launch_pick_best(const uint32_t* records, uint32_t count, unsigned long long index_base, const double* params,
                      bool first_chunk, BestPick* pick, BestPickHost* pick_host, hipStream_t st,
                      uint32_t* records_host = nullptr ,
                      uint32_t* best_count = nullptr );
void launch_lead_fold_keep(const uint32_t* counts_rep, uint32_t rep_stride, uint32_t lead, const uint8_t* valid,
                           uint32_t h_count, uint32_t* records, uint32_t* best_count, const uint32_t* ub,
                           unsigned long long* keep, uint32_t n_groups_rest, hipStream_t st,
                           uint32_t* records_dev = nullptr,
                           uint32_t group_begin = 0xFFFFFFFFu ,
                           unsigned long long* pick_key = nullptr ,
                           unsigned long long* pick_key2 = nullptr ,
                           uint32_t* surv_count = nullptr, uint32_t* surv = nullptr ,
                           const RefHistArgs* ref = nullptr );
void launch_count_bits(const unsigned long long* masks, const unsigned long long* keep, uint32_t n_tiles,
                       uint32_t n_groups, unsigned long long* total, hipStream_t st);

}
```

### misc3d_amd/csrc/m3d_fit.cpp

```cpp
#include "m3d_driver_internal.hpp"
#include "m3d_generalfit_fp.hpp"

#pragma clang fp contract(off)

namespace m3d {

static uint64_t double_to_size_t_x86(double v) {
    const double two63 = 9223372036854775808.0;
    if (v >= two63) {
        const double w = v - two63;
        if (!(w < two63)) return 0;
        return static_cast<uint64_t>(static_cast<int64_t>(w)) ^ 0x8000000000000000ull;
    }
    if (!(v > -two63)) return 0x8000000000000000ull;
    return static_cast<uint64_t>(static_cast<int64_t>(v));
}

template <class TieFn, class BestFn>
static void replay_range(m3d_replay_state* st, size_t n_points, int kind, size_t max_iteration,
                         double probability, size_t begin, size_t end, const uint8_t* valid,
                         const uint32_t* counts, TieFn tie, BestFn on_best) {
    const bool packed = valid == nullptr;
    const int m = minimal_sample(kind);
    for (size_t i = begin; i < end; ++i) {
// ... 55 lines not shown
        const uint32_t want = mx | 0x80000000u;
        for (size_t k = 0; k < n; ++k) {
            if (rec[k] != want) continue;
            const size_t i = begin + k;
            const double fitness = (double)mx / (double)n_points;
            bool better = fitness > st->best_fitness;
            double trial_rmse = 0.0;
            bool trial_rmse_known = false;
            if (!better && fitness == st->best_fitness) better = tie(i, mx, &trial_rmse, &trial_rmse_known);
            if (better) {
                st->best_fitness = fitness;
                st->best_rmse = trial_rmse;
                st->best_rmse_known = trial_rmse_known ? 1 : 0;
                st->best_index = (int64_t)i;
                st->best_count = mx;
                on_best(i);
                st->current_iteration = (uint64_t)max_iteration;
            }
        }
    }
    st->count += nvalid;
    st->iterations = end;
}

struct SampleSource {
    Mt19937Mod rng;
    size_t n_points = 0;
    const uint32_t* table = nullptr;
    int m = 3;
    void seed(uint64_t s) { rng.seed((uint32_t)(s & 0xffffffffull)); }
    void fill(size_t begin, size_t end, uint32_t* out) {
        if (table) {
            std::memcpy(out, table + begin * m, sizeof(uint32_t) * (end - begin) * m);
            return;
        }
        if (rng.d != (uint32_t)n_points) rng.set_modulus((uint32_t)n_points);
        const size_t n = end - begin;
        if (m == 3) rng.fill<3>(out, n);
        else if (m == 2) rng.fill<2>(out, n);
        else rng.fill<4>(out, n);
    }
};

static uint32_t pick_splits(uint32_t n_tiles, uint32_t h_pad) {
    const uint32_t groups = h_pad / 64;
    const uint32_t target_wgs = (uint32_t)config().dense_workgroups;
    const uint32_t want = std::max<uint32_t>(1, (target_wgs + n_tiles - 1) / n_tiles);
    return std::min(want, groups);
}

static thread_local int t_dense_fit = 0;
static bool use_dense_scoring() { return t_dense_fit != 0 || config().dense_scoring != 0; }

static uint32_t lead_size() { return (uint32_t)config().lead_hypotheses; }

static size_t chunk_cap_for(const CloudView& v, const SortedView& sv, size_t times = 1) {
    if (!use_dense_scoring()) {
        const size_t by_masks = sv.n_tiles ? std::max<size_t>(((size_t)1 << 30) / ((size_t)sv.n_tiles * 8), 16) * 64 : ~(size_t)0;
        return std::min<size_t>(std::min<size_t>((size_t)config().chunk_cap * times, 262144), by_masks);
    }
    const uint32_t rows = std::max<uint32_t>(1, v.n_pad / kScoreTile);
    const size_t cap = std::min<size_t>(16384, ((size_t)1 << 28) / rows / 64 * 64);
    return std::max<size_t>(cap, 64);
}

static bool bound_pays(uint32_t n_tiles, size_t window_hypotheses) {
    return window_hypotheses >= 8192 && (double)n_tiles * (double)window_hypotheses >= 1.5e7;
}
static int bound_mode(int kind) {
    const int mode = config().plane_bound;
    return (mode != 0 && kind == M3D_PLANE && config().ref_bound == 2) ? 2 : mode;
}

static bool prestream_enabled() { return config().prestream != 0; }
static int pre_stream_gate(DeviceCtx* ctx) {
    if (!pre_stream_of(ctx) || !ctx->ev_pre_gate) return M3D_OK;
    HIPCHK(hipEventRecord(ctx->ev_pre_gate, ctx->stream));
    HIPCHK(hipStreamWaitEvent(ctx->pre_stream, ctx->ev_pre_gate, 0));
    return M3D_OK;
}

constexpr size_t kBoundTicketWords = 8192;
static int reserve_survivor_scratch(DeviceCtx* ctx, uint32_t h_pad) {
    const size_t words = kBoundTicketWords + (size_t)h_pad + 64;
    if ((size_t)h_pad / 64 + 2 > kBoundTicketWords) return fail(M3D_ERR_INTERNAL, "window too large for the bound's tickets");
    if (ctx->surv_list.cap < sizeof(uint32_t) * words) {
        RESERVE(ctx->surv_list, sizeof(uint32_t) * (kBoundTicketWords + 2 * ((size_t)h_pad + 64)));
        HIPCHK(hipMemsetAsync(ctx->surv_list.p, 0, ctx->surv_list.cap, ctx->stream));
    }
    return M3D_OK;
}
static uint32_t* bound_tickets(DeviceCtx* ctx) { return ctx->surv_list.as<uint32_t>(); }
static uint32_t* bound_list(DeviceCtx* ctx) { return ctx->surv_list.as<uint32_t>() + kBoundTicketWords; }

static int issue_chunk(DeviceCtx* ctx, ChunkSlot& s, const CloudView& v, const SortedView& sv, int kind,
                       double thr, size_t begin, size_t end, SampleSource& src, double* ms_sample,
                       bool prune = false, uint32_t lead = 0, bool new_fit = false ,
                       bool device_records = false ,
                       m3d_comm* comm = nullptr,
                       bool caller_ships_records = false ,
                       const PickFinal* pick_final = nullptr ,
                       bool nothing_to_prune = false ,
                       bool pre = false ,
                       const double* move_best_from = nullptr ,
                       bool first_of_stream = false ,
                       SegmentRounds* rounds = nullptr ) {
    const bool kill_rides = rounds && rounds->poison_pending && kind == M3D_PLANE;
    const int m = minimal_sample(kind);
    const uint32_t count = (uint32_t)(end - begin);
    const bool dense = use_dense_scoring();
    pre = pre && !dense && prune && !new_fit && !comm && lead == 0 && !(rounds && rounds->poison_pending) && ctx->pre_stream && s.pre_done;
    hipStream_t st_pre = pre ? ctx->pre_stream : ctx->stream;
    if (move_best_from)
        HIPCHK(hipMemcpyAsync(ctx->best_params.p, move_best_from, sizeof(double) * kModelStride, hipMemcpyDeviceToDevice, st_pre));
    const bool timing = config().kernel_timing != 0;
    if (comm && dense) return fail(M3D_ERR_INVALID_ARG, "sharded fits use the culled scoring path (m3d_config.dense_scoring = 0)");
    const uint32_t world = comm ? (uint32_t)comm->world : 1u, rank = comm ? (uint32_t)comm->rank : 0u;
    const uint32_t sl_pad = round_up((count + world - 1) / world, 64);
    const uint32_t h_pad = comm ? sl_pad * world : round_up(count, 64);
    const uint32_t n_tiles = v.n_pad / kScoreTile;
    if (comm) device_records = true;
    s.begin = begin;
    s.end = end;
    s.h_pad = h_pad;
    RESERVE(s.samples, sizeof(uint32_t) * (size_t)count * m);
    RESERVE(s.score, sizeof(double) * kModelStride * ((size_t)h_pad + 1));
    RESERVE(s.params, sizeof(double) * kModelStride * ((size_t)h_pad + 1));
    RESERVE(s.valid, (size_t)h_pad + 1);
    Cull32Out c32;
    const bool cull32 = !dense && config().cull_fp32 != 0 && sv.radius < 1e18;
    if (cull32) {
        RESERVE(s.cull32, sizeof(float) * 24 * ((size_t)h_pad / 2 + 1));
        c32.out = s.cull32.as<float>();
        for (int k = 0; k < 3; ++k) c32.origin[k] = sv.origin[k];
        c32.radius = sv.radius;
    }
    if (dense || device_records) RESERVE(s.counts, sizeof(uint32_t) * ((size_t)h_pad + 1));
    uint32_t* rec_dev = (!dense && device_records) ? s.counts.as<uint32_t>() : nullptr;
    RESERVE(s.h_samples, sizeof(uint32_t) * (size_t)count * m);
    RESERVE(s.h_counts, sizeof(uint32_t) * ((size_t)h_pad + 4));
    RESERVE(s.h_valid, (size_t)h_pad + 1);
    if (dense) {
        RESERVE(ctx->partial, sizeof(uint32_t) * (size_t)n_tiles * h_pad);
    } else {
        RESERVE(s.masks, sizeof(uint64_t) * (size_t)std::max<uint32_t>(sv.n_tiles, 1) * (h_pad / 64));
        RESERVE(ctx->keep, sizeof(uint64_t) * (size_t)(h_pad / 64));
        RESERVE(ctx->counts_rep, sizeof(uint32_t) * ((size_t)kCountReplicas * h_pad + kPairReplicas));
    }
    const double t0 = now_ms();
    src.fill(begin, end, s.h_samples.as<uint32_t>());
    if (ms_sample) *ms_sample += now_ms() - t0;
    if (!dense && prune) RESERVE(s.ub, sizeof(uint32_t) * 3 * (size_t)h_pad);
    const bool use_lead = !dense && prune && lead >= 64 && lead % 64 == 0 && lead + 64 <= count && (!comm || sl_pad >= lead + 64);
    const bool own_real_ = !comm || (size_t)rank * sl_pad < count;
    LeadPrep lp;
    const bool lead_prepared = use_lead && new_fit && own_real_ && lead <= h_pad && (uint32_t)kPairReplicas <= h_pad;
    const bool all_prepared = nothing_to_prune && !use_lead && lead == 0 && !dense && prune && new_fit && !comm &&
                              (uint32_t)kPairReplicas <= h_pad;
    if (lead_prepared || all_prepared) {
        lp.counts_rep = ctx->counts_rep.as<uint32_t>();
        lp.keep = ctx->keep.as<unsigned long long>();
        lp.rep_stride = h_pad;
        lp.n_rep = kCountReplicas;
        lp.n_lead = all_prepared ? h_pad : lead;
        lp.n_pair = kPairReplicas;
    }
    const bool fit_launched =
        launch_minimal_fit(kind, v, s.h_samples.as<uint32_t>(), count, h_pad + 1, thr, s.score.as<double>(),
                       s.params.as<double>(), s.valid.as<uint8_t>(), st_pre,
                       (!dense && prune) ? s.ub.as<uint32_t>() : nullptr,
                       new_fit ? ctx->best_count.as<uint32_t>() : nullptr, (lead_prepared || all_prepared) ? &lp : nullptr, sv.max_abs,
                       cull32 ? &c32 : nullptr, kill_rides ? &rounds->pending_poison : nullptr,
                       (!dense && prune) ? s.ub.as<uint32_t>() + h_pad : nullptr);
    if (fit_launched && kill_rides) {
        rounds->poison_pending = false;
        if (rounds->poison_expected_at) *rounds->poison_expected_at += rounds->poison_pending_count;
    }
    if (dense)
        HIPCHK(hipMemsetAsync(s.counts.p, 0, sizeof(uint32_t) * (size_t)h_pad, ctx->stream));
    s.lead_groups = 0;
    s.lead_fused = false;
    s.scored = false;
    s.poll_seq = 0;
    s.host_has_records = true;
    s.done_on_copy_stream = false;
    uint32_t* h_pairs = s.h_counts.as<uint32_t>() + h_pad;
    if (dense) {
        HIPCHK(hipEventRecord(s.k0, ctx->stream));
        launch_score(kind, v, s.score.as<double>(), h_pad, pick_splits(n_tiles, h_pad),
                     ctx->partial.as<uint32_t>(), ctx->stream);
        HIPCHK(hipEventRecord(s.k1, ctx->stream));
        launch_reduce_partials(ctx->partial.as<uint32_t>(), n_tiles, h_pad, s.counts.as<uint32_t>(),
                               ctx->stream);
        s.scored = true;
    } else {
        const uint32_t n_groups = h_pad / 64;
        const uint32_t g0 = comm ? rank * (sl_pad / 64) : 0u, g1 = comm ? g0 + sl_pad / 64 : n_groups;
        const bool own_real = (size_t)g0 * 64 < count;
        uint32_t* ub = prune ? s.ub.as<uint32_t>() : nullptr;
        uint32_t* ubp = (prune && (use_lead || !new_fit) && c32.out && !sv.has_dead && score_phases_for(kind) != 0) ? ub + h_pad : nullptr;
        auto* masks = s.masks.as<unsigned long long>();
        auto* keep = ctx->keep.as<unsigned long long>();
        uint32_t* pair_rep = ctx->counts_rep.as<uint32_t>() + (size_t)kCountReplicas * h_pad;
        uint32_t* bc = prune ? ctx->best_count.as<uint32_t>() : nullptr;
        const bool solo = comm && comm->world == 1 && comm->transport == m3d_comm::kRccl;
        uint32_t* rec_host = (comm && !solo) ? nullptr : s.h_counts.as<uint32_t>();
        PickFinal pfin;
        if (pick_final) {
            pfin = *pick_final;
            pfin.params = s.params.as<double>();
        }
        const uint32_t ga = use_lead ? lead / 64 : 0u;
        if (own_real) {
            s.lead_fused = false;
            if (ga && g0 == 0 && c32.out) {
                if (!lead_prepared)
                    launch_keep_mask(ub, bc, ga, keep, ctx->stream, ctx->counts_rep.as<uint32_t>(), h_pad, 0);
                s.lead_fused = launch_cull_lead(kind, sv, s.score.as<double>(), c32.out, masks, keep, n_groups, ga,
                                                ctx->counts_rep.as<uint32_t>(), h_pad, pair_rep, ub, g1, ctx->stream, ubp);
            }
            const bool bound_on = (kind == M3D_CYLINDER || !ubp) && prune && bc && sv.frames && bound_mode(kind) != 0 &&
                                  (bound_mode(kind) == 2 || (kind != M3D_SPHERE && bound_pays(sv.n_tiles, comm ? sl_pad : count))) &&
                                  (use_lead || !new_fit) && std::max(g0, ga) < g1;
            const bool ref_on = bound_on && kind == M3D_PLANE && !ubp && !comm && (new_fit || first_of_stream) && use_lead && ga && g0 == 0 && !sv.has_dead &&
                                config().ref_bound != 0 && (config().ref_bound == 2 || bound_pays(sv.n_tiles, count));
            RefHistArgs ref;
            if (ref_on) {
                RESERVE(ctx->ref_hist, ref_hist_bytes(sv.n_tiles));
                ref.sx = sv.x; ref.sy = sv.y; ref.sz = sv.z;
                ref.n_tiles = sv.n_tiles;
                ref.score = s.score.as<double>();
                ref.counts_rep = ctx->counts_rep.as<uint32_t>();
                ref.rep_stride = h_pad;
                ref.lead = lead;
                ref.valid = s.valid.as<uint8_t>();
                ref.h_count = count;
                ref.max_abs = sv.max_abs;
                ref.min_count = config().ref_bound == 2 ? 1u : 8u * sv.n_tiles;
                ref_hist_place(ref, ctx->ref_hist.p);
            }
            uint32_t* const ubsum = ubp ? ub + 2 * (size_t)h_pad : ub + h_pad;
            if (bound_on) {
                const int src = reserve_survivor_scratch(ctx, h_pad);
                if (src != M3D_OK) return src;
                if (ubp) HIPCHK(hipMemsetAsync(ubsum, 0, sizeof(uint32_t) * h_pad, ctx->stream));
            }
            uint32_t* const surv_count = bound_on ? bc + 6 : nullptr;
            uint32_t* const surv = bound_on ? bound_list(ctx) : nullptr;
            unsigned long long* touched = nullptr;
            bool touched_written = false;
            if (bound_on && kind == M3D_CYLINDER && c32.out && !s.lead_fused && !(ga && g0 >= ga) && g1 - g0 >= 128u) {
                RESERVE(s.touched, sizeof(uint64_t) * (size_t)((sv.n_tiles + 63u) / 64u) * h_pad);
                touched = s.touched.as<unsigned long long>();
            }
            if (!s.lead_fused) {
                if (ga && g0 >= ga)
                    launch_cull_mask(kind, sv, s.score.as<double>(), s.valid.as<uint8_t>(), count, n_groups, masks, ub,
                                     ctx->stream, true, 0, ga, c32.out);
                launch_cull_mask(kind, sv, s.score.as<double>(), s.valid.as<uint8_t>(), count, n_groups, masks, ub, st_pre,
                                 true, g0, g1, c32.out, ubp, touched, h_pad, &touched_written);
            }
            if (pre) {
                HIPCHK(hipEventRecord(s.pre_done, ctx->pre_stream));
                HIPCHK(hipStreamWaitEvent(ctx->stream, s.pre_done, 0));
            }
            uint32_t g_lo = g0;
            if (ga) {
                s.lead_groups = ga;
                g_lo = std::max(g0, ga);
                if (!s.lead_fused) {
                    if (!lead_prepared)
                        launch_keep_mask(ub, bc, ga, keep, ctx->stream, ctx->counts_rep.as<uint32_t>(), h_pad, 0);
                    launch_score_mask(kind, sv, s.score.as<double>(), masks, keep, n_groups, ctx->counts_rep.as<uint32_t>(),
                                      h_pad, pair_rep, ctx->stream, 0, ga, timing ? s.k2 : nullptr, timing ? s.k3 : nullptr);
                }
                launch_lead_fold_keep(ctx->counts_rep.as<uint32_t>(), h_pad, lead, s.valid.as<uint8_t>(), count,
                                      g0 == 0 ? rec_host : nullptr, bc, ub, keep, g1 - g_lo, ctx->stream,
                                      g0 == 0 ? rec_dev : nullptr, g_lo, pick_final ? pick_final->key : nullptr,
                                      pick_final ? pick_final->key2 : nullptr, surv_count, surv, ref_on ? &ref : nullptr);
            } else if (!all_prepared) {
                launch_keep_mask(ub, bc, g1 - g0, keep, ctx->stream, ctx->counts_rep.as<uint32_t>(), h_pad, g0, surv_count, surv);
            }
            if (bound_on)
                launch_plane_bound(kind, sv, s.score.as<double>(), masks, keep, n_groups, g_lo, g1, ubsum, bc, surv_count, surv,
                                   bound_tickets(ctx), c32.out, ctx->stream, bound_mode(kind) == 2,
                                   touched_written && g_lo == g0 ? touched : nullptr, h_pad, ref_on ? &ref : nullptr);
            bool phased = false;
            if (ubp)
                phased = launch_score_phased(kind, sv, s.score.as<double>(), masks, keep, n_groups, ctx->counts_rep.as<uint32_t>(), h_pad,
                                             pair_rep, ub, ubp, bc, ctx->stream, g_lo, g1, timing ? s.k0 : nullptr, timing ? s.k1 : nullptr);
            if (!phased)
                launch_score_mask(kind, sv, s.score.as<double>(), masks, keep, n_groups, ctx->counts_rep.as<uint32_t>(), h_pad,
                                  pair_rep, ctx->stream, g_lo, g1, timing ? s.k0 : nullptr, timing ? s.k1 : nullptr, bound_on);
            launch_sum_replicas(ctx->counts_rep.as<uint32_t>(), h_pad, g1 * 64u, rec_host, pair_rep, h_pairs,
                                s.valid.as<uint8_t>(), count, bc, ctx->stream, g_lo * 64u, rec_dev, pick_final ? &pfin : nullptr,
                                phased ? keep : nullptr);
            if (pick_final) s.poll_seq = pick_final->seq;
            s.scored = timing;
        } else {
            HIPCHK(hipMemsetAsync(rec_dev + (size_t)g0 * 64, 0, sizeof(uint32_t) * sl_pad, ctx->stream));
            h_pairs[0] = h_pairs[1] = h_pairs[2] = 0;
        }
        if (solo) {
            comm->collectives++;
            s.host_has_records = true;
        } else if (comm) {
            int host_has_all = 0;
            const int rc = comm->allgather_u32_device(rec_dev, sl_pad, ctx->stream, s.h_counts.as<uint32_t>(), &host_has_all);
            if (rc != M3D_OK) return rc;
            s.host_has_records = host_has_all != 0;
            if (!host_has_all && caller_ships_records) {
                HIPCHK(hipEventRecord(ctx->ev_compact, ctx->stream));
                HIPCHK(hipStreamWaitEvent(copy_stream_of(ctx), ctx->ev_compact, 0));
                HIPCHK(hipMemcpyAsync(s.h_counts.p, rec_dev, sizeof(uint32_t) * (size_t)count, hipMemcpyDeviceToHost,
                                      copy_stream_of(ctx)));
                HIPCHK(hipGetLastError());
                HIPCHK(hipEventRecord(s.done, copy_stream_of(ctx)));
                s.host_has_records = true;
                s.done_on_copy_stream = true;
                return M3D_OK;
            }
            if (!host_has_all && !caller_ships_records) {
                HIPCHK(hipMemcpyAsync(s.h_counts.p, rec_dev, sizeof(uint32_t) * (size_t)count, hipMemcpyDeviceToHost,
                                      ctx->stream));
                s.host_has_records = true;
            }
        }
    }
    if (dense)
        HIPCHK(hipMemcpyAsync(s.h_counts.p, s.counts.p, sizeof(uint32_t) * (size_t)count, hipMemcpyDeviceToHost,
                              ctx->stream));
    if (dense) HIPCHK(hipMemcpyAsync(s.h_valid.p, s.valid.p, (size_t)count, hipMemcpyDeviceToHost, ctx->stream));
    HIPCHK(hipGetLastError());
    if (!caller_ships_records && !s.poll_seq) HIPCHK(hipEventRecord(s.done, ctx->stream));
    return M3D_OK;
}

static int wait_pick_seq(DeviceCtx* ctx, uint32_t seq) {
    const volatile uint32_t* p = &ctx->h_pick.as<BestPickHost>()->seq;
    const int spin_us = std::max(config().wait_spin_us, 30);
    const auto t0 = std::chrono::steady_clock::now();
    bool sleeping = false;
    for (uint32_t spins = 1;; ++spins) {
        if ((int32_t)(*p - seq) >= 0) break;
        if (sleeping) {
            std::this_thread::sleep_for(std::chrono::microseconds(20));
            if ((spins & 0x3Fu) == 0) {
                const hipError_t q = hipStreamQuery(ctx->stream);
                if (q == hipSuccess) {
                    if ((int32_t)(*p - seq) >= 0) break;
                    return fail(M3D_ERR_INTERNAL, "the scoring chunk finished without its completion word");
                }
                if (q != hipErrorNotReady) return fail(M3D_ERR_DEVICE, std::string("hipStreamQuery: ") + hipGetErrorString(q));
            }
            continue;
        }
        if ((spins & 0xFFu) == 0 &&
            std::chrono::duration_cast<std::chrono::microseconds>(std::chrono::steady_clock::now() - t0).count() >= spin_us)
            sleeping = true;
#if defined(__x86_64__) || defined(__i386__)
        __builtin_ia32_pause();
#endif
    }
    std::atomic_thread_fence(std::memory_order_acquire);
    return M3D_OK;
}

int stream_wait_spin(DeviceCtx* ctx) {
    const int spin_us = config().wait_spin_us;
    if (spin_us <= 0) {
        HIPCHK(hipStreamSynchronize(ctx->stream));
        return M3D_OK;
    }
    if (!ctx->h_sync.p) {
        RESERVE(ctx->h_sync, 64);
        std::memset(ctx->h_sync.p, 0, 64);
    }
    if (++ctx->sync_seq == 0) ++ctx->sync_seq;
    const uint32_t seq = ctx->sync_seq;
// ... 752 lines not shown
m3d_sampler* m3d_sampler_create(size_t n_points, int kind, uint64_t seed) {
    if (kind < 0 || kind > 2 || n_points < (size_t)minimal_sample(kind) || n_points >= ((size_t)1 << 31)) {
        set_error("m3d_sampler_create: invalid argument");
        return nullptr;
    }
    m3d_sampler* s = new m3d_sampler();
    s->kind = kind;
    s->src.seed(seed);
    s->src.n_points = n_points;
    s->src.m = minimal_sample(kind);
    return s;
}
void m3d_sampler_destroy(m3d_sampler* s) { delete s; }
size_t m3d_sampler_drawn(const m3d_sampler* s) { return s ? s->drawn : 0; }
const uint32_t* m3d_sampler_table(m3d_sampler* s, size_t n_hypotheses) {
    if (!s) return nullptr;
    s->draw_until(n_hypotheses);
    return s->table.data();
}

int m3d_cloud_score_shard(m3d_cloud* c, m3d_sampler* sampler, double threshold, size_t begin, size_t end,
                          size_t slice, uint32_t world, uint32_t rank, uint32_t* counts, uint8_t* valid,
                          size_t* n_mine) {
    if (!c || !sampler || !counts || !n_mine || end < begin || slice == 0 || world == 0 || rank >= world)
        return fail(M3D_ERR_INVALID_ARG, "invalid argument");
    const int kind = sampler->kind;
    if (kind == M3D_CYLINDER && !c->has_normals)
        return fail(M3D_ERR_NO_NORMALS, "Fit cylinder requires normals.");
    if (sampler->src.n_points != c->n) return fail(M3D_ERR_INVALID_ARG, "sampler and cloud sizes differ");
    if (sampler->drawn > begin) return fail(M3D_ERR_INVALID_ARG, "sampler is already past `begin`");
    DeviceCtx* ctx = c->ctx;
    CtxLock lock(ctx);
    HIPCHK(hipSetDevice(ctx->device));
    {
        const int frc = ensure_plane_frames(c, kind, end - begin);
        if (frc != M3D_OK) return frc;
    }
    const CloudView v = c->view();
    const SortedView sv = c->sorted();
    const size_t chunk_cap = chunk_cap_for(v, sv);
    SampleSource tsrc;
    tsrc.m = sampler->src.m;
    size_t out = 0;
    struct Pending {
        bool active = false, discard = false;
        size_t out_pos = 0, n = 0;
    } pend[2];
    int cur = 0;
    auto collect = [&](int k) -> int {
        if (!pend[k].active) return M3D_OK;
        ChunkSlot& s = ctx->slot[k];
        HIPCHK(hipEventSynchronize(s.done));
        if (!pend[k].discard) {
            if (valid) {
                unpack_slot(s);
                std::memcpy(counts + pend[k].out_pos, s.h_counts.p, sizeof(uint32_t) * pend[k].n);
                std::memcpy(valid + pend[k].out_pos, s.h_valid.p, pend[k].n);
            } else if (!use_dense_scoring()) {
                std::memcpy(counts + pend[k].out_pos, s.h_counts.p, sizeof(uint32_t) * pend[k].n);
            } else {
                const uint32_t* hc = s.h_counts.as<uint32_t>();
                const uint8_t* hv = s.h_valid.as<uint8_t>();
                for (size_t i = 0; i < pend[k].n; ++i)
                    counts[pend[k].out_pos + i] = hc[i] | (hv[i] ? 0x80000000u : 0u);
            }
        }
        pend[k].active = pend[k].discard = false;
        return M3D_OK;
    };
    size_t j = 0;
    bool first_piece = true;
    const bool prestream_on = prestream_enabled();
    constexpr size_t kFirstPiece = 2048;
    bool first_own = true;
    if (prestream_on && !use_dense_scoring()) {
        const int grc = pre_stream_gate(ctx);
        if (grc != M3D_OK) return grc;
    }
    RESERVE(ctx->best_count, 32);
    RESERVE(ctx->h_inc, 64);
    if (begin == 0) sampler->incumbent = 0;
    *ctx->h_inc.as<uint32_t>() = sampler->incumbent;
    HIPCHK(hipMemcpyAsync(ctx->best_count.p, ctx->h_inc.p, sizeof(uint32_t), hipMemcpyHostToDevice, ctx->stream));
    HIPCHK(hipMemsetAsync(ctx->best_count.as<uint32_t>() + 6, 0, sizeof(uint32_t), ctx->stream));
    {
        const size_t first_own = begin + (size_t)rank * slice;
        if (rank > 0 && first_own < end) {
            const size_t w = std::min<size_t>(std::min<size_t>(lead_size(), chunk_cap), first_own - begin);
            sampler->draw_until(begin + w);
            tsrc.table = sampler->table.data();
            const int rc = issue_chunk(ctx, ctx->slot[cur], v, sv, kind, threshold, begin, begin + w, tsrc, nullptr, true);
            if (rc != M3D_OK) return rc;
            pend[cur].active = pend[cur].discard = true;
            pend[cur].n = w;
            cur ^= 1;
            first_piece = false;
        }
    }
    for (size_t b = begin; b < end; b += slice, ++j) {
        const size_t e = std::min(end, b + slice);
        if (j % world != rank) {
            sampler->draw_until(e);
            continue;
        }
        for (size_t bb = b; bb < e;) {
            const uint32_t lead = first_piece ? lead_size() : 0u;
            first_piece = false;
            const bool short_first = first_own && e - bb > chunk_cap && kFirstPiece >= 2 * (size_t)lead_size();
            const size_t ee = std::min(e, bb + (short_first ? kFirstPiece : chunk_cap));
            const bool pre = prestream_on && !first_own && lead == 0;
            first_own = false;
            sampler->draw_until(ee);
            int rc = collect(cur);
            if (rc != M3D_OK) return rc;
            tsrc.table = sampler->table.data();
            rc = issue_chunk(ctx, ctx->slot[cur], v, sv, kind, threshold, bb, ee, tsrc, nullptr, true, lead, false, false, nullptr, false,
                             nullptr, false, pre, nullptr, world == 1 && bb == 0);
            if (rc != M3D_OK) return rc;
            pend[cur].active = true;
            pend[cur].out_pos = out;
            pend[cur].n = ee - bb;
            out += ee - bb;
            cur ^= 1;
            bb = ee;
        }
    }
    int rc = collect(0);
    if (rc != M3D_OK) return rc;
    rc = collect(1);
    if (rc != M3D_OK) return rc;
    HIPCHK(hipMemcpyAsync(ctx->h_inc.p, ctx->best_count.p, sizeof(uint32_t), hipMemcpyDeviceToHost, ctx->stream));
    HIPCHK(hipStreamSynchronize(ctx->stream));
    sampler->incumbent = *ctx->h_inc.as<uint32_t>();
    *n_mine = out;
    return M3D_OK;
}

int m3d_bench_time_score(m3d_cloud* c, int kind, double threshold, const uint32_t* samples,
                         size_t n_hypotheses, int reps, int mode, double* ms_avg, uint64_t* listed_pairs) {
    if (!c || kind < 0 || kind > 2 || !samples || !ms_avg || reps < 1 || n_hypotheses == 0 ||
        n_hypotheses > 16384 || mode < 0 || mode > 2)
        return fail(M3D_ERR_INVALID_ARG, "invalid argument");
    if (kind == M3D_CYLINDER && !c->has_normals)
        return fail(M3D_ERR_NO_NORMALS, "Fit cylinder requires normals.");
    DeviceCtx* ctx = c->ctx;
    CtxLock lock(ctx);
    HIPCHK(hipSetDevice(ctx->device));
    const CloudView v = c->view();
    const SortedView sv = c->sorted();
    SampleSource src;
    src.table = samples;
    src.m = minimal_sample(kind);
    ChunkSlot& s = ctx->slot[0];
    int rc = issue_chunk(ctx, s, v, sv, kind, threshold, 0, n_hypotheses, src, nullptr);
    if (rc != M3D_OK) return rc;
    const uint32_t count = (uint32_t)n_hypotheses;
    const uint32_t n_tiles = v.n_pad / kScoreTile;
    RESERVE(ctx->partial, sizeof(uint32_t) * (size_t)n_tiles * s.h_pad);
    const uint32_t n_groups = s.h_pad / 64;
    RESERVE(ctx->masks, sizeof(uint64_t) * (size_t)std::max<uint32_t>(sv.n_tiles, 1) * n_groups);
    RESERVE(ctx->keep, sizeof(uint64_t) * (size_t)n_groups);
    RESERVE(ctx->counts_rep, sizeof(uint32_t) * ((size_t)kCountReplicas * s.h_pad + kPairReplicas));
    RESERVE(ctx->small, 256);
    auto* masks = ctx->masks.as<unsigned long long>();
    auto* keep = ctx->keep.as<unsigned long long>();
    const float* c32 = (!use_dense_scoring() && config().cull_fp32 != 0 && sv.radius < 1e18) ? s.cull32.as<float>() : nullptr;
    launch_cull_mask(kind, sv, s.score.as<double>(), s.valid.as<uint8_t>(), count, n_groups, masks, nullptr, ctx->stream, false, 0,
// ... 22 lines not shown
    HIPCHK(hipGetLastError());
    HIPCHK(hipStreamSynchronize(ctx->stream));
    float ms = 0;
    HIPCHK(hipEventElapsedTime(&ms, ctx->ev0, ctx->ev1));
    *ms_avg = (double)ms / reps;
    return M3D_OK;
}

int m3d_bench_upper_bounds(m3d_cloud* c, int kind, double threshold, const uint32_t* samples, size_t n_hypotheses, uint32_t* ub_out);
int m3d_bench_plane_upper_bounds(m3d_cloud* c, double threshold, const uint32_t* samples, size_t n_hypotheses, uint32_t* ub_out) {
    return m3d_bench_upper_bounds(c, M3D_PLANE, threshold, samples, n_hypotheses, ub_out);
}
static int bench_upper_bounds(m3d_cloud* c, int kind, double threshold, const uint32_t* samples, size_t n_hypotheses, uint32_t* ub_out,
                              long ref_index);
int m3d_bench_upper_bounds(m3d_cloud* c, int kind, double threshold, const uint32_t* samples, size_t n_hypotheses, uint32_t* ub_out) {
    return bench_upper_bounds(c, kind, threshold, samples, n_hypotheses, ub_out, -1);
}
int m3d_bench_plane_ref_upper_bounds(m3d_cloud* c, double threshold, const uint32_t* samples, size_t n_hypotheses, size_t ref_index,
                                     uint32_t* ub_out) {
    if (ref_index >= n_hypotheses) return fail(M3D_ERR_INVALID_ARG, "invalid argument");
    return bench_upper_bounds(c, M3D_PLANE, threshold, samples, n_hypotheses, ub_out, (long)ref_index);
}
static int bench_upper_bounds(m3d_cloud* c, int kind, double threshold, const uint32_t* samples, size_t n_hypotheses, uint32_t* ub_out,
                              long ref_index) {
    if (!c || !samples || !ub_out || n_hypotheses == 0 || n_hypotheses > 16384 || kind < M3D_PLANE || kind > M3D_CYLINDER)
        return fail(M3D_ERR_INVALID_ARG, "invalid argument");
    if (kind == M3D_CYLINDER && !c->has_normals) return fail(M3D_ERR_INVALID_ARG, "cylinder hypotheses need normals");
    DeviceCtx* ctx = c->ctx;
    CtxLock lock(ctx);
    HIPCHK(hipSetDevice(ctx->device));
    if (c->work.active || c->n_tiles == 0) return fail(M3D_ERR_INVALID_ARG, "the cloud has no sorted copy of its own");
    if (!c->frames_ready) {
        if (!c->frames.reserve(sizeof(double) * kFrameStride * (size_t)c->n_tiles) ||
            !c->frame_cum.reserve(sizeof(uint16_t) * kCumStride * (size_t)c->n_tiles))
            return fail(M3D_ERR_DEVICE, "out of device memory (tile frames)");
        launch_tile_frames(c->sorted(), c->frames.as<double>(), c->frame_cum.as<uint16_t>(), ctx->stream);
        c->frames_ready = true;
    }
    const CloudView v = c->view();
    const SortedView sv = c->sorted();
    SampleSource src;
    src.table = samples;
    src.m = (uint32_t)minimal_sample(kind);
    ChunkSlot& s = ctx->slot[0];
    int rc = issue_chunk(ctx, s, v, sv, kind, threshold, 0, n_hypotheses, src, nullptr);
    if (rc != M3D_OK) return rc;
    const uint32_t n_groups = s.h_pad / 64;
    RESERVE(ctx->masks, sizeof(uint64_t) * (size_t)std::max<uint32_t>(sv.n_tiles, 1) * n_groups);
    RESERVE(ctx->keep, sizeof(uint64_t) * (size_t)n_groups);
    RESERVE(ctx->small, 256);
    RESERVE(s.ub, sizeof(uint32_t) * 3 * (size_t)s.h_pad);
    rc = reserve_survivor_scratch(ctx, s.h_pad);
    if (rc != M3D_OK) return rc;
    auto* masks = ctx->masks.as<unsigned long long>();
    auto* keep = ctx->keep.as<unsigned long long>();
    uint32_t* ubsum = s.ub.as<uint32_t>() + s.h_pad;
    uint32_t* ctl = ctx->small.as<uint32_t>();
    uint32_t* surv = bound_list(ctx);
    const float* c32 = (!use_dense_scoring() && config().cull_fp32 != 0 && sv.radius < 1e18) ? s.cull32.as<float>() : nullptr;
    HIPCHK(hipMemsetAsync(ubsum, 0, sizeof(uint32_t) * (size_t)s.h_pad, ctx->stream));
    HIPCHK(hipMemsetAsync(ctl, 0, 8, ctx->stream));
    launch_cull_mask(kind, sv, s.score.as<double>(), s.valid.as<uint8_t>(), (uint32_t)n_hypotheses, n_groups, masks, nullptr,
                     ctx->stream, false, 0, 0xFFFFFFFFu, c32);
    launch_keep_mask(nullptr, nullptr, n_groups, keep, ctx->stream, nullptr, 0, 0, ctl + 1, surv);
    RefHistArgs ref;
    if (ref_index >= 0) {
        RESERVE(ctx->ref_hist, ref_hist_bytes(sv.n_tiles));
        ref.sx = sv.x; ref.sy = sv.y; ref.sz = sv.z;
        ref.n_tiles = sv.n_tiles;
        ref.score = s.score.as<double>();
        ref.fixed_index = (uint32_t)ref_index;
        ref.max_abs = sv.max_abs;
        ref_hist_place(ref, ctx->ref_hist.p);
        launch_ref_hist(ref, ctx->stream);
    }
    launch_plane_bound(kind, sv, s.score.as<double>(), masks, keep, n_groups, 0, n_groups, ubsum, ctl, ctl + 1, surv,
                       bound_tickets(ctx), c32, ctx->stream, true, nullptr, 0, ref_index >= 0 ? &ref : nullptr, true);
    HIPCHK(hipMemcpyAsync(ub_out, ubsum, sizeof(uint32_t) * n_hypotheses, hipMemcpyDeviceToHost, ctx->stream));
    HIPCHK(hipGetLastError());
    HIPCHK(hipStreamSynchronize(ctx->stream));
    return M3D_OK;
}


}
```

Baseline: 60.88 million.

## Have plane bound emit a compact survivor list and score only listed hypotheses

The plane upper-bound kernel now writes the ids of hypotheses that survive the bound into a compact final list, using a wave ballot and an atomic append. The scoring path can then run over that list instead of walking the whole keep mask. The shared tile-load and screen-batch logic is factored into reusable device functions for a new list-driven score kernel. This is meant to cut wasted work on masked-out hypothesis groups, at the cost of extra atomics, a doubled survivor scratch buffer, and a length word that must be reset by the replica-summing kernel.

Result: no change. 60.41 million (-0.8%).

```diff
diff --git a/include/misc3d_amd.h b/include/misc3d_amd.h
--- a/include/misc3d_amd.h
+++ b/include/misc3d_amd.h
@@ -466,6 +466,7 @@
     int32_t list_mask;
     int32_t mask_early;
     int32_t ref_bound;
+    int32_t score_list;
 } m3d_config;
 void m3d_get_config(m3d_config *out);
 int m3d_set_config(const m3d_config *in);
diff --git a/include/misc3d_amd_bench.h b/include/misc3d_amd_bench.h
--- a/include/misc3d_amd_bench.h
+++ b/include/misc3d_amd_bench.h
@@ -22,6 +22,8 @@
                                      size_t ref_index, uint32_t *ub_out);
 int m3d_bench_upper_bounds(m3d_cloud *cloud, int kind, double threshold, const uint32_t *samples, size_t n_hypotheses,
                            uint32_t *ub_out);
+int m3d_bench_score_list(m3d_cloud *cloud, double threshold, const uint32_t *samples, size_t n_hypotheses, const uint32_t *ids,
+                         size_t n_ids, uint32_t *counts_out);
 int m3d_bench_last_segment_ms(double out[6]);
 
 int m3d_bench_reg_checkers(const double *ps, const double *pd, const double *T, double edge_threshold,
diff --git a/misc3d_amd/capi.py b/misc3d_amd/capi.py
--- a/misc3d_amd/capi.py
+++ b/misc3d_amd/capi.py
@@ -258,7 +258,7 @@
                                          "reg_neighbour_lists", "reg_prune", "match_brute", "match_fp32_screen",
                                          "pool_limit_mb", "kernel_timing", "reg_sorted_lists", "score_fp32_screen",
                                          "cull_fp32", "reg_fp32_screen", "sorted_tombstones", "score_mfma", "score_mfma_groups", "score_waves4", "score_waves4_groups", "score_phases", "compact_one_pass", "plane_bound",
-                                         "lanes", "wait_spin_us", "prestream", "chunk_cap", "first_chunk", "reg_cells_per_radius", "match_pipeline", "reg_cache", "device_aliases", "lanes_eager", "list_mask", "mask_early", "ref_bound")]
+                                         "lanes", "wait_spin_us", "prestream", "chunk_cap", "first_chunk", "reg_cells_per_radius", "match_pipeline", "reg_cache", "device_aliases", "lanes_eager", "list_mask", "mask_early", "ref_bound", "score_list")]
 
 
 def fp64_issue_rate(device=0, ms_target=2.0):
@@ -658,6 +658,15 @@
         _check(lib().m3d_bench_upper_bounds(self._h, kind, threshold, _p(samples), len(samples), _p(ub)))
         return ub
 
+    def bench_score_list(self, threshold, samples, ids):
+        samples = np.ascontiguousarray(samples, dtype=np.uint32).reshape(-1, 3)
+        ids = np.ascontiguousarray(ids, dtype=np.uint32).reshape(-1)
+        cnt = np.zeros(len(samples), dtype=np.uint32)
+        f = lib().m3d_bench_score_list
+        f.argtypes = [C.c_void_p, C.c_double, C.c_void_p, C.c_size_t, C.c_void_p, C.c_size_t, C.c_void_p]
+        _check(f(self._h, threshold, _p(samples), len(samples), _p(ids), len(ids), _p(cnt)))
+        return cnt
+
     def exact_error(self, kind, threshold, model):
         model = _f64(model)
         cnt = C.c_uint64(0)
diff --git a/misc3d_amd/csrc/m3d_bound.hip b/misc3d_amd/csrc/m3d_bound.hip
--- a/misc3d_amd/csrc/m3d_bound.hip
+++ b/misc3d_amd/csrc/m3d_bound.hip
@@ -216,7 +216,8 @@
                                                                    uint32_t* __restrict__ ubsum, const uint32_t* __restrict__ best_count,
                                                                    unsigned long long* __restrict__ keep,
                                                                    uint32_t* __restrict__ tickets ,
-                                                                   uint32_t max_list, RefHistArgs ref, bool ref_alone) {
+                                                                   uint32_t max_list, RefHistArgs ref, bool ref_alone,
+                                                                   FinalList fin ) {
     constexpr int kBoundTpb = kBoundWaves * kBoundTpw;
     constexpr int kRefTpb = REF ? kBoundTpb : 1;
     static_assert(!REF || KIND == 0, "reference histograms bound planes");
@@ -233,7 +234,10 @@
     const int wave = __builtin_amdgcn_readfirstlane((int)(threadIdx.x >> 6));
     const uint32_t total = surv_count[0];
     if (total > max_list) {
-        if (blockIdx.x == 0 && blockIdx.y == 0 && threadIdx.x == 0) surv_count[0] = 0u;
+        if (blockIdx.x == 0 && blockIdx.y == 0 && threadIdx.x == 0) {
+            if (fin.len) fin.len[0] = kFinalListIsKept | total;
+            surv_count[0] = 0u;
+        }
         return;
     }
     if (blockIdx.x * 64u >= total) return;
@@ -364,7 +368,16 @@
                 __threadfence();
                 const uint32_t best = best_count[0];
                 const uint32_t sum = has ? atomicAdd(&ubsum[h], 0u) : 0u;
-                if (has && best != 0u && sum < best) atomicAnd(&keep[h >> 6], ~bit);
+                const bool stays = has && !(best != 0u && sum < best);
+                if (has && !stays) atomicAnd(&keep[h >> 6], ~bit);
+                if (fin.len) {
+                    const unsigned long long sm = __ballot(stays);
+                    uint32_t fbase = 0;
+                    if (lane == 0 && sm) fbase = atomicAdd(fin.len, (uint32_t)__popcll(sm));
+                    fbase = (uint32_t)__builtin_amdgcn_readfirstlane((int)fbase);
+                    const uint32_t frank = __builtin_amdgcn_mbcnt_hi((uint32_t)(sm >> 32), __builtin_amdgcn_mbcnt_lo((uint32_t)sm, 0u));
+                    if (stays) fin.ids[fbase + frank] = h;
+                }
                 uint32_t done = 0;
                 if (lane == 0) {
                     tickets[1u + blk] = 0u;
@@ -466,7 +479,7 @@
                         uint32_t n_groups, uint32_t group_begin, uint32_t group_end, uint32_t* ubsum,
                         const uint32_t* best_count, uint32_t* surv_count, const uint32_t* surv, uint32_t* tickets,
                         const float* cull32, hipStream_t st, bool always, const unsigned long long* touched, uint32_t touched_stride,
-                        const RefHistArgs* ref, bool ref_alone) {
+                        const RefHistArgs* ref, bool ref_alone, FinalList fin) {
     group_end = std::min(group_end, n_groups);
     if (!s.frames || !s.frame_cum || !s.n_tiles || !surv || !surv_count || !tickets || group_begin >= group_end) return;
     const uint32_t window = group_end - group_begin;
@@ -485,7 +498,7 @@
     if (s.radius >= 1e18 || kind == 1) cull32 = nullptr;
     auto go = [&](auto kernel) {
         kernel<<<g, b, 0, st>>>(s.frames, s.frame_cum, s.n_tiles, s.max_abs, score, masks, n_groups, s.boxes, cull32, surv_count, surv,
-                                ubsum, best_count, keep, tickets, max_list, (ref && kind == 0) ? *ref : RefHistArgs{}, ref_alone);
+                                ubsum, best_count, keep, tickets, max_list, (ref && kind == 0) ? *ref : RefHistArgs{}, ref_alone, fin);
     };
     if (kind == 0 && ref) go(plane_bound_k<0, tpw, true>);
     else if (kind == 0) go(plane_bound_k<0, tpw, false>);
diff --git a/misc3d_amd/csrc/m3d_config.cpp b/misc3d_amd/csrc/m3d_config.cpp
--- a/misc3d_amd/csrc/m3d_config.cpp
+++ b/misc3d_amd/csrc/m3d_config.cpp
@@ -51,6 +51,7 @@
     if (c.list_mask > 16) c.list_mask = 16;
     c.mask_early = c.mask_early != 0;
     if (c.ref_bound < 0 || c.ref_bound > 2) c.ref_bound = 1;
+    if (c.score_list < 0 || c.score_list > 2) c.score_list = 1;
 }
 void load_env() {
     std::memset(&g_cfg, 0, sizeof(g_cfg));
@@ -86,6 +87,7 @@
     g_cfg.list_mask = (int32_t)env_long("M3D_LIST_MASK", 1);
     g_cfg.mask_early = !env_is("M3D_MASK_EARLY", '0');
     g_cfg.ref_bound = (int32_t)env_long("M3D_REF_BOUND", 1);
+    g_cfg.score_list = (int32_t)env_long("M3D_SCORE_LIST", 1);
     sanitize(g_cfg);
 }
 }
diff --git a/misc3d_amd/csrc/m3d_cull_kernels.hip b/misc3d_amd/csrc/m3d_cull_kernels.hip
--- a/misc3d_amd/csrc/m3d_cull_kernels.hip
+++ b/misc3d_amd/csrc/m3d_cull_kernels.hip
@@ -740,6 +740,163 @@
     m = mn;
 }
 
+template <int KIND, int Q>
+__device__ __forceinline__ void screen_tile_load(const double* __restrict__ sx, const double* __restrict__ sy, const double* __restrict__ sz,
+                                                 const double* __restrict__ boxes, const float* __restrict__ tile_f32, uint32_t has_dead,
+                                                 uint32_t tile, int lane, double (&box)[6], f32x2 (&xf)[Q], f32x2 (&yf)[Q], f32x2 (&zf)[Q],
+                                                 f32x2 (&wf)[Q] , uint32_t& dead8, bool& tile_screened,
+                                                 bool& tile_has_dead) {
+    const size_t base = (size_t)tile * kTilePoints + lane;
+#pragma unroll
+    for (int k = 0; k < 6; ++k) box[k] = boxes[(size_t)tile * kBoxStride + k];
+    if (tile_f32) {
+        const f32x2* __restrict__ t2 = reinterpret_cast<const f32x2*>(tile_f32 + (size_t)tile * kTileF32Floats) + lane;
+#pragma unroll
+        for (int j = 0; j < Q; ++j) {
+            xf[j] = t2[(0 * Q + j) * 64];
+            yf[j] = t2[(1 * Q + j) * 64];
+            zf[j] = t2[(2 * Q + j) * 64];
+        }
+        tile_screened = boxes[(size_t)tile * kBoxStride + 6] != 0.0;
+    } else {
+        float chk = 0.0f;
+#pragma unroll
+        for (int j = 0; j < Q; ++j) {
+            xf[j] = {(float)(sx[base + 128 * j] - box[0]), (float)(sx[base + 128 * j + 64] - box[0])};
+            yf[j] = {(float)(sy[base + 128 * j] - box[1]), (float)(sy[base + 128 * j + 64] - box[1])};
+            zf[j] = {(float)(sz[base + 128 * j] - box[2]), (float)(sz[base + 128 * j + 64] - box[2])};
+            chk += ((xf[j].x + xf[j].y) + (yf[j].x + yf[j].y)) + (zf[j].x + zf[j].y);
+        }
+        tile_screened = __ballot(!(chk * 0.0f == 0.0f)) == 0ull;
+    }
+    if (KIND == 1) {
+#pragma unroll
+        for (int j = 0; j < Q; ++j) {
+            f32x2 w = xf[j] * xf[j];
+            w = __builtin_elementwise_fma(yf[j], yf[j], w);
+            wf[j] = __builtin_elementwise_fma(zf[j], zf[j], w);
+        }
+    }
+    dead8 = 0;
+    tile_has_dead = false;
+    if (KIND == 0 && has_dead && tile_f32) {
+#pragma unroll
+        for (int j = 0; j < Q; ++j) dead8 = (dead8 << 2) | (xf[j].x != xf[j].x ? 2u : 0u) | (xf[j].y != xf[j].y ? 1u : 0u);
+        tile_has_dead = tile_screened && __ballot(dead8 != 0u) != 0ull;
+    }
+}
+
+template <int KIND, int Q>
+__device__ __forceinline__ void screen_batch(const double* __restrict__ sx, const double* __restrict__ sy, const double* __restrict__ sz,
+                                             const double* __restrict__ score, double max_abs, uint32_t* __restrict__ counts,
+                                             uint32_t* __restrict__ pair_rep, uint32_t tile, int lane, const double (&box)[6],
+                                             const f32x2 (&xf)[Q], const f32x2 (&yf)[Q], const f32x2 (&zf)[Q], const f32x2 (&wf)[Q],
+                                             uint32_t dead8, bool tile_screened, bool tile_has_dead, const int my, const uint32_t nb) {
+    __shared__ __attribute__((aligned(16))) uint8_t cnt8[64 * kCntStride];
+    constexpr int NL = KIND == 2 ? 3 : 2;
+    __shared__ float4 loc[64 + 1][NL];
+    constexpr int P = 2 * Q;
+    const size_t base = (size_t)tile * kTilePoints + lane;
+    auto exact_count = [&](uint32_t id) -> uint32_t {
+        double rec[kModelStride];
+        const double* __restrict__ rp = score + (size_t)id * kModelStride;
+#pragma unroll
+        for (int k = 0; k < kModelStride; ++k) rec[k] = rp[k];
+        uint32_t c = 0;
+#pragma unroll 1
+        for (int half = 0; half < 2; ++half) {
+            double x[P / 2], y[P / 2], z[P / 2];
+#pragma unroll
+            for (int j = 0; j < P / 2; ++j) {
+                x[j] = sx[base + 64 * (half * (P / 2) + j)];
+                y[j] = sy[base + 64 * (half * (P / 2) + j)];
+                z[j] = sz[base + 64 * (half * (P / 2) + j)];
+            }
+            c += tile_count<KIND, P / 2>(rec, x, y, z);
+        }
+        return c;
+    };
+    {
+        const double* __restrict__ rp = score + (size_t)my * kModelStride;
+        constexpr int kRec = KIND == 2 ? 8 : 5;
+        double rec[kRec];
+#pragma unroll
+        for (int k = 0; k < kRec; ++k) rec[k] = rp[k];
+        float sr[12];
+        if (KIND == 0) plane_screen_record(rec, box, max_abs, sr);
+        else if (KIND == 1) sphere_screen_record(rec, box, max_abs, sr);
+        else cylinder_screen_record(rec, box, max_abs, sr);
+        loc[lane][0] = make_float4(sr[0], sr[1], sr[2], sr[3]);
+        loc[lane][1] = make_float4(sr[4], sr[5], sr[6], sr[7]);
+        if (KIND == 2) loc[lane][NL - 1] = make_float4(sr[8], sr[9], sr[10], sr[11]);
+    }
+    __syncthreads();
+    uint32_t park = 0;
+    auto step = [&](auto screened, auto dead, const float4 ra, const float4 rb, const float4 rc, uint32_t k, uint8_t* cnt_row) {
+        constexpr bool SCREENED = decltype(screened)::value;
+        constexpr bool DEAD = decltype(dead)::value;
+        uint32_t bits = 0;
+        bool exact = true;
+        if (SCREENED) {
+            float m;
+            screen_eval<KIND, Q>(ra, rb, rc, xf, yf, zf, wf, bits, m);
+            if (DEAD) bits &= ~dead8;
+            exact = __ballot(!(m >= (KIND == 0 ? rb.y : (KIND == 1 ? rb.w : rc.z)))) != 0ull;
+        }
+        if (__builtin_expect(exact, 0)) {
+            const uint32_t e = exact_count((uint32_t)__builtin_amdgcn_readlane(my, (int)k));
+            if (lane == 0) atomicAdd(&pair_rep[(uint32_t)kPairMain + tile % (uint32_t)(kPairLead - kPairMain)], 1u);
+            park = ((uint32_t)lane == k) ? e : park;
+            bits = 0;
+        }
+        *cnt_row = (uint8_t)bits;
+    };
+    auto batch = [&](auto screened, auto dead) {
+        uint32_t rec_off = 0, cnt_off = (uint32_t)lane;
+        asm volatile("" : "+v"(rec_off), "+v"(cnt_off));
+        const char* const loc_b = reinterpret_cast<const char*>(&loc[0][0]);
+        auto fetch = [&](int i, float4& r0, float4& r1, float4& r2) {
+            const float4* __restrict__ r = reinterpret_cast<const float4*>(loc_b + rec_off) + i * NL;
+            r0 = r[0];
+            r1 = r[1];
+            r2 = r[NL - 1];
+            __builtin_amdgcn_sched_barrier(0);
+        };
+        float4 a0, a1, a2, b0r, b1r, b2r;
+        fetch(0, a0, a1, a2);
+        for (uint32_t k = 0; k < nb; k += 4u) {
+            fetch(1, b0r, b1r, b2r);
+            step(screened, dead, a0, a1, a2, k, cnt8 + cnt_off);
+            fetch(2, a0, a1, a2);
+            if (k + 1u < nb) step(screened, dead, b0r, b1r, b2r, k + 1u, cnt8 + cnt_off + kCntStride);
+            fetch(3, b0r, b1r, b2r);
+            if (k + 2u < nb) step(screened, dead, a0, a1, a2, k + 2u, cnt8 + cnt_off + 2 * kCntStride);
+            fetch(4, a0, a1, a2);
+            if (k + 3u < nb) step(screened, dead, b0r, b1r, b2r, k + 3u, cnt8 + cnt_off + 3 * kCntStride);
+            rec_off += 4u * NL * (uint32_t)sizeof(float4);
+            cnt_off += 4u * kCntStride;
+        }
+    };
+    if (tile_screened && !tile_has_dead) batch(std::true_type{}, std::false_type{});
+    else if (tile_screened) batch(std::true_type{}, std::true_type{});
+    else batch(std::false_type{}, std::false_type{});
+    __syncthreads();
+    if ((uint32_t)lane < nb) {
+        const uint4* row = reinterpret_cast<const uint4*>(cnt8 + (uint32_t)lane * kCntStride);
+        uint32_t sum = park;
+#pragma unroll
+        for (int i = 0; i < 4; ++i) {
+            const uint4 v = row[i];
+            sum += (uint32_t)__popc(v.x);
+            sum += (uint32_t)__popc(v.y);
+            sum += (uint32_t)__popc(v.z);
+            sum += (uint32_t)__popc(v.w);
+        }
+        if (sum) atomicAdd(&counts[(uint32_t)my], sum);
+    }
+    __syncthreads();
+}
+
 template <int KIND, bool OWN_BOX_TESTS>
 __device__ __forceinline__ void score_screen_body(const double* __restrict__ sx, const double* __restrict__ sy,
                                                   const double* __restrict__ sz,
@@ -754,9 +911,6 @@
                                                   const float* __restrict__ cull32, const float* __restrict__ tile_f32,
                                                   uint32_t has_dead ) {
     __shared__ uint16_t ids[kScreenMaxGroups * 64];
-    __shared__ __attribute__((aligned(16))) uint8_t cnt8[64 * kCntStride];
-    constexpr int NL = KIND == 2 ? 3 : 2;
-    __shared__ float4 loc[64 + 1][NL];
     const int lane = threadIdx.x & 63;
     const uint32_t tile = block_x;
     uint32_t* __restrict__ counts = counts_rep + (size_t)(tile % kCountReplicas) * rep_stride;
@@ -780,49 +934,12 @@
         mm = masks[(size_t)tile * n_groups + g0 + lane] & keep[g0 + lane];
     }
     if (!__ballot(mm != 0)) return;
-    const size_t base = (size_t)tile * kTilePoints + lane;
-    constexpr int P = kTilePoints / 64, Q = P / 2;
+    constexpr int Q = kTilePoints / 128;
     double box[6];
-#pragma unroll
-    for (int k = 0; k < 6; ++k) box[k] = boxes[(size_t)tile * kBoxStride + k];
-    f32x2 xf[Q], yf[Q], zf[Q];
-    bool tile_screened;
-    if (tile_f32) {
-        const f32x2* __restrict__ t2 = reinterpret_cast<const f32x2*>(tile_f32 + (size_t)tile * kTileF32Floats) + lane;
-#pragma unroll
-        for (int j = 0; j < Q; ++j) {
-            xf[j] = t2[(0 * Q + j) * 64];
-            yf[j] = t2[(1 * Q + j) * 64];
-            zf[j] = t2[(2 * Q + j) * 64];
-        }
-        tile_screened = boxes[(size_t)tile * kBoxStride + 6] != 0.0;
-    } else {
-        float chk = 0.0f;
-#pragma unroll
-        for (int j = 0; j < Q; ++j) {
-            xf[j] = {(float)(sx[base + 128 * j] - box[0]), (float)(sx[base + 128 * j + 64] - box[0])};
-            yf[j] = {(float)(sy[base + 128 * j] - box[1]), (float)(sy[base + 128 * j + 64] - box[1])};
-            zf[j] = {(float)(sz[base + 128 * j] - box[2]), (float)(sz[base + 128 * j + 64] - box[2])};
-            chk += ((xf[j].x + xf[j].y) + (yf[j].x + yf[j].y)) + (zf[j].x + zf[j].y);
-        }
-        tile_screened = __ballot(!(chk * 0.0f == 0.0f)) == 0ull;
-    }
-    f32x2 wf[Q];
-    if (KIND == 1) {
-#pragma unroll
-        for (int j = 0; j < Q; ++j) {
-            f32x2 w = xf[j] * xf[j];
-            w = __builtin_elementwise_fma(yf[j], yf[j], w);
-            wf[j] = __builtin_elementwise_fma(zf[j], zf[j], w);
-        }
-    }
-    uint32_t dead8 = 0;
-    bool tile_has_dead = false;
-    if (KIND == 0 && has_dead && tile_f32) {
-#pragma unroll
-        for (int j = 0; j < Q; ++j) dead8 = (dead8 << 2) | (xf[j].x != xf[j].x ? 2u : 0u) | (xf[j].y != xf[j].y ? 1u : 0u);
-        tile_has_dead = tile_screened && __ballot(dead8 != 0u) != 0ull;
-    }
+    f32x2 xf[Q], yf[Q], zf[Q], wf[Q];
+    uint32_t dead8;
+    bool tile_screened, tile_has_dead;
+    screen_tile_load<KIND, Q>(sx, sy, sz, boxes, tile_f32, has_dead, tile, lane, box, xf, yf, zf, wf, dead8, tile_screened, tile_has_dead);
     uint32_t total = 0;
     const int mm_lo = (int)(uint32_t)mm, mm_hi = (int)(uint32_t)(mm >> 32);
     for (uint32_t w = 0; w < groups_per_block; ++w) {
@@ -835,108 +952,11 @@
     }
     __syncthreads();
     if (threadIdx.x == 0) atomicAdd(&pair_rep[(tile + block_y * 67u) % (uint32_t)kPairMain], total);
-    const double* __restrict__ score0 = score + (size_t)g0 * 64u * kModelStride;
-    auto exact_count = [&](uint32_t id) -> uint32_t {
-        double rec[kModelStride];
-        const double* __restrict__ rp = score0 + (size_t)id * kModelStride;
-#pragma unroll
-        for (int k = 0; k < kModelStride; ++k) rec[k] = rp[k];
-        uint32_t c = 0;
-#pragma unroll 1
-        for (int half = 0; half < 2; ++half) {
-            double x[P / 2], y[P / 2], z[P / 2];
-#pragma unroll
-            for (int j = 0; j < P / 2; ++j) {
-                x[j] = sx[base + 64 * (half * (P / 2) + j)];
-                y[j] = sy[base + 64 * (half * (P / 2) + j)];
-                z[j] = sz[base + 64 * (half * (P / 2) + j)];
-            }
-            c += tile_count<KIND, P / 2>(rec, x, y, z);
-        }
-        return c;
-    };
     for (uint32_t b0 = 0; b0 < total; b0 += 64u) {
         const uint32_t nb = min(64u, total - b0);
-        const int my = (b0 + (uint32_t)lane < total) ? (int)ids[b0 + lane] : 0;
-        {
-            const double* __restrict__ rp = score0 + (size_t)my * kModelStride;
-            constexpr int kRec = KIND == 2 ? 8 : 5;
-            double rec[kRec];
-#pragma unroll
-            for (int k = 0; k < kRec; ++k) rec[k] = rp[k];
-            float sr[12];
-            if (KIND == 0) plane_screen_record(rec, box, max_abs, sr);
-            else if (KIND == 1) sphere_screen_record(rec, box, max_abs, sr);
-            else cylinder_screen_record(rec, box, max_abs, sr);
-            loc[lane][0] = make_float4(sr[0], sr[1], sr[2], sr[3]);
-            loc[lane][1] = make_float4(sr[4], sr[5], sr[6], sr[7]);
-            if (KIND == 2) loc[lane][NL - 1] = make_float4(sr[8], sr[9], sr[10], sr[11]);
-        }
-        __syncthreads();
-        uint32_t park = 0;
-        auto step = [&](auto screened, auto dead, const float4 ra, const float4 rb, const float4 rc, uint32_t k, uint8_t* cnt_row) {
-            constexpr bool SCREENED = decltype(screened)::value;
-            constexpr bool DEAD = decltype(dead)::value;
-            uint32_t bits = 0;
-            bool exact = true;
-            if (SCREENED) {
-                float m;
-                screen_eval<KIND, Q>(ra, rb, rc, xf, yf, zf, wf, bits, m);
-                if (DEAD) bits &= ~dead8;
-                exact = __ballot(!(m >= (KIND == 0 ? rb.y : (KIND == 1 ? rb.w : rc.z)))) != 0ull;
-            }
-            if (__builtin_expect(exact, 0)) {
-                const uint32_t e = exact_count((uint32_t)__builtin_amdgcn_readlane(my, (int)k));
-                if (lane == 0) atomicAdd(&pair_rep[(uint32_t)kPairMain + tile % (uint32_t)(kPairLead - kPairMain)], 1u);
-                park = ((uint32_t)lane == k) ? e : park;
-                bits = 0;
-            }
-            *cnt_row = (uint8_t)bits;
-        };
-        auto batch = [&](auto screened, auto dead) {
-            uint32_t rec_off = 0, cnt_off = (uint32_t)lane;
-            asm volatile("" : "+v"(rec_off), "+v"(cnt_off));
-            const char* const loc_b = reinterpret_cast<const char*>(&loc[0][0]);
-            auto fetch = [&](int i, float4& r0, float4& r1, float4& r2) {
-                const float4* __restrict__ r = reinterpret_cast<const float4*>(loc_b + rec_off) + i * NL;
-                r0 = r[0];
-                r1 = r[1];
-                r2 = r[NL - 1];
-                __builtin_amdgcn_sched_barrier(0);
-            };
-            float4 a0, a1, a2, b0r, b1r, b2r;
-            fetch(0, a0, a1, a2);
-            for (uint32_t k = 0; k < nb; k += 4u) {
-                fetch(1, b0r, b1r, b2r);
-                step(screened, dead, a0, a1, a2, k, cnt8 + cnt_off);
-                fetch(2, a0, a1, a2);
-                if (k + 1u < nb) step(screened, dead, b0r, b1r, b2r, k + 1u, cnt8 + cnt_off + kCntStride);
-                fetch(3, b0r, b1r, b2r);
-                if (k + 2u < nb) step(screened, dead, a0, a1, a2, k + 2u, cnt8 + cnt_off + 2 * kCntStride);
-                fetch(4, a0, a1, a2);
-                if (k + 3u < nb) step(screened, dead, b0r, b1r, b2r, k + 3u, cnt8 + cnt_off + 3 * kCntStride);
-                rec_off += 4u * NL * (uint32_t)sizeof(float4);
-                cnt_off += 4u * kCntStride;
-            }
-        };
-        if (tile_screened && !tile_has_dead) batch(std::true_type{}, std::false_type{});
-        else if (tile_screened) batch(std::true_type{}, std::true_type{});
-        else batch(std::false_type{}, std::false_type{});
-        __syncthreads();
-        if ((uint32_t)lane < nb) {
-            const uint4* row = reinterpret_cast<const uint4*>(cnt8 + (uint32_t)lane * kCntStride);
-            uint32_t sum = park;
-#pragma unroll
-            for (int i = 0; i < 4; ++i) {
-                const uint4 v = row[i];
-                sum += (uint32_t)__popc(v.x);
-                sum += (uint32_t)__popc(v.y);
-                sum += (uint32_t)__popc(v.z);
-                sum += (uint32_t)__popc(v.w);
-            }
-            if (sum) atomicAdd(&counts[g0 * 64u + (uint32_t)my], sum);
-        }
-        __syncthreads();
+        const int my = (b0 + (uint32_t)lane < total) ? (int)(g0 * 64u + ids[b0 + lane]) : 0;
+        screen_batch<KIND, Q>(sx, sy, sz, score, max_abs, counts, pair_rep, tile, lane, box, xf, yf, zf, wf, dead8, tile_screened,
+                              tile_has_dead, my, nb);
     }
 }
 __device__ __forceinline__ uint32_t phase_tile4(uint32_t bx, uint32_t res_mask) {
@@ -966,6 +986,78 @@
                                    blockIdx.y, nullptr, tile_f32, has_dead);
 }
 
+constexpr uint32_t kListPerSplit = 32, kListMinSplits = 2, kListFetch = 4;
+__device__ __forceinline__ uint32_t list_splits(uint32_t len, uint32_t max_splits) {
+    return min(max((len + kListPerSplit - 1u) / kListPerSplit, kListMinSplits), max_splits);
+}
+template <int KIND>
+__global__ __launch_bounds__(64) void score_list_k(const double* __restrict__ sx, const double* __restrict__ sy,
+                                                    const double* __restrict__ sz, const double* __restrict__ boxes, double max_abs,
+                                                    const double* __restrict__ score, const unsigned long long* __restrict__ masks,
+                                                    uint32_t n_groups, uint32_t* __restrict__ counts_rep, uint32_t rep_stride,
+                                                    uint32_t* __restrict__ pair_rep, const float* __restrict__ tile_f32,
+                                                    uint32_t has_dead, uint32_t n_tiles, const uint32_t* __restrict__ list_len,
+                                                    const uint32_t* __restrict__ list_final, const uint32_t* __restrict__ list_kept) {
+    __shared__ uint32_t ids[64 + 64 * kListFetch];
+    const uint32_t tile = blockIdx.x;
+    if (tile >= n_tiles) return;
+    const uint32_t word = list_len[0];
+    const uint32_t len = word & ~kFinalListIsKept;
+    const uint32_t splits = list_splits(len, gridDim.y);
+    if (blockIdx.y >= splits || len == 0u) return;
+    const uint32_t* __restrict__ list = (word & kFinalListIsKept) ? list_kept : list_final;
+    const uint32_t begin = (uint32_t)(((uint64_t)len * blockIdx.y) / splits), end = (uint32_t)(((uint64_t)len * (blockIdx.y + 1u)) / splits);
+    const int lane = threadIdx.x & 63;
+    uint32_t* __restrict__ counts = counts_rep + (size_t)(tile % kCountReplicas) * rep_stride;
+    const unsigned long long* __restrict__ mrow = masks + (size_t)tile * n_groups;
+    constexpr int Q = kTilePoints / 128;
+    uint32_t pos = begin, n = 0, off = 0, pairs = 0;
+    auto gather = [&]() {
+        while (n < 64u && pos < end) {
+            uint32_t h[kListFetch];
+            unsigned long long w[kListFetch];
+#pragma unroll
+            for (uint32_t u = 0; u < kListFetch; ++u) {
+                const uint32_t p = pos + 64u * u + (uint32_t)lane;
+                h[u] = p < end ? list[p] : 0xFFFFFFFFu;
+            }
+#pragma unroll
+            for (uint32_t u = 0; u < kListFetch; ++u) w[u] = h[u] != 0xFFFFFFFFu ? mrow[h[u] >> 6] : 0ull;
+#pragma unroll
+            for (uint32_t u = 0; u < kListFetch; ++u) {
+                const bool pass = ((w[u] >> (h[u] & 63u)) & 1ull) != 0ull;
+                const unsigned long long pm = __ballot(pass);
+                if (pass) ids[n + __builtin_amdgcn_mbcnt_hi((uint32_t)(pm >> 32), __builtin_amdgcn_mbcnt_lo((uint32_t)pm, 0u))] = h[u];
+                n += (uint32_t)__popcll(pm);
+            }
+            pos += 64u * kListFetch;
+        }
+    };
+    gather();
+    if (n == 0u) return;
+    double box[6];
+    f32x2 xf[Q], yf[Q], zf[Q], wf[Q];
+    uint32_t dead8;
+    bool tile_screened, tile_has_dead;
+    screen_tile_load<KIND, Q>(sx, sy, sz, boxes, tile_f32, has_dead, tile, lane, box, xf, yf, zf, wf, dead8, tile_screened, tile_has_dead);
+    do {
+        __syncthreads();
+        const uint32_t nb = min(n, 64u);
+        const int my = (uint32_t)lane < nb ? (int)ids[off + lane] : 0;
+        screen_batch<KIND, Q>(sx, sy, sz, score, max_abs, counts, pair_rep, tile, lane, box, xf, yf, zf, wf, dead8, tile_screened,
+                              tile_has_dead, my, nb);
+        pairs += nb;
+        n -= nb;
+        off += nb;
+        if (n < 64u && pos < end) {
+            if ((uint32_t)lane < n) ids[lane] = ids[off + lane];
+            off = 0;
+            gather();
+        }
+    } while (n != 0u);
+    if (threadIdx.x == 0) atomicAdd(&pair_rep[(tile + blockIdx.y * 67u) % (uint32_t)kPairMain], pairs);
+}
+
 __global__ __launch_bounds__(64) void phase_keep_k(const uint32_t* __restrict__ counts_rep, uint32_t rep_stride,
                                                     const uint32_t* __restrict__ ub, const uint32_t* __restrict__ ubp,
                                                     const uint32_t* __restrict__ best_count_ptr,
@@ -1014,8 +1106,10 @@
                                uint32_t* __restrict__ pairs_out, const uint8_t* __restrict__ valid, uint32_t h_count,
                                uint32_t* __restrict__ best_count, uint32_t h_begin,
                                uint32_t* __restrict__ counts_dev , PickFinal pf,
-                               const unsigned long long* __restrict__ keep_final ) {
+                               const unsigned long long* __restrict__ keep_final ,
+                               uint32_t* __restrict__ consumed_list_len ) {
     const uint32_t h = h_begin + blockIdx.x * 256u + threadIdx.x;
+    if (consumed_list_len && blockIdx.x == 0 && threadIdx.x == 0) consumed_list_len[0] = 0u;
     if (blockIdx.x == 0 && pair_rep && pairs_out) {
         __shared__ uint32_t red[256];
         uint32_t p = 0;
@@ -1121,13 +1215,13 @@
 void launch_sum_replicas(const uint32_t* counts_rep, uint32_t rep_stride, uint32_t h_end, uint32_t* counts,
                          const uint32_t* pair_rep, uint32_t* pairs_out, const uint8_t* valid, uint32_t h_count,
                          uint32_t* best_count, hipStream_t st, uint32_t h_begin, uint32_t* counts_dev, const PickFinal* pick,
-                         const unsigned long long* keep_final) {
+                         const unsigned long long* keep_final, uint32_t* consumed_list_len) {
     PickFinal pf;
     if (pick) pf = *pick;
     if (h_end > h_begin)
         sum_replicas_k<<<(h_end - h_begin + 255) / 256, 256, 0, st>>>(counts_rep, rep_stride, h_end, counts, pair_rep,
                                                                       pairs_out, valid, h_count, best_count, h_begin,
-                                                                      counts_dev, pf, keep_final);
+                                                                      counts_dev, pf, keep_final, consumed_list_len);
 }
 
 bool launch_cull_lead(int kind, const SortedView& s, const double* score, const float* cull32, unsigned long long* masks,
@@ -1226,13 +1320,36 @@
                                     records_host, best_count);
 }
 
+bool score_list_applies(int kind) { return kind == 0 && config().score_list != 0 && config().score_fp32_screen != 0; }
+void launch_score_list(const SortedView& s, const double* score, const unsigned long long* masks, uint32_t n_groups,
+                       uint32_t* counts_rep, uint32_t rep_stride, uint32_t* pair_rep, hipStream_t st, uint32_t window_groups,
+                       FinalList list, hipEvent_t ev_start, hipEvent_t ev_stop) {
+    if (!s.n_tiles || !window_groups || !list.len) return;
+    const uint32_t gpb_max = screen_gpb_max(window_groups, true);
+    const uint32_t min_wgs = (uint32_t)config().score_min_workgroups;
+    const uint32_t gpb = std::max<uint32_t>(1, std::min<uint32_t>(gpb_max, (uint32_t)(((uint64_t)s.n_tiles * window_groups) / min_wgs)));
+    const dim3 g((s.n_tiles + 7u) / 8u * 8u, std::max<uint32_t>((window_groups + gpb - 1) / gpb, 2u)), b(64);
+    const uint32_t* kept = list.kept ? list.kept : list.ids;
+    if (ev_start && ev_stop)
+        hipExtLaunchKernelGGL(score_list_k<0>, g, b, 0, st, ev_start, ev_stop, 0, s.x, s.y, s.z, s.boxes, s.max_abs, score, masks, n_groups,
+                              counts_rep, rep_stride, pair_rep, (const float*)s.tile_f32, s.has_dead ? 1u : 0u, s.n_tiles,
+                              (const uint32_t*)list.len, (const uint32_t*)list.ids, kept);
+    else
+        score_list_k<0><<<g, b, 0, st>>>(s.x, s.y, s.z, s.boxes, s.max_abs, score, masks, n_groups, counts_rep, rep_stride, pair_rep,
+                                         (const float*)s.tile_f32, s.has_dead ? 1u : 0u, s.n_tiles, list.len, list.ids, kept);
+}
+
 void launch_score_mask(int kind, const SortedView& s, const double* score, const unsigned long long* masks,
                        const unsigned long long* keep, uint32_t n_groups, uint32_t* counts_rep, uint32_t rep_stride,
                        uint32_t* pair_rep, hipStream_t st, uint32_t group_begin, uint32_t group_end, hipEvent_t ev_start,
-                       hipEvent_t ev_stop, bool thinned) {
+                       hipEvent_t ev_stop, bool thinned, FinalList list) {
     group_end = std::min(group_end, n_groups);
     if (!s.n_tiles || group_begin >= group_end) return;
     const uint32_t window = group_end - group_begin;
+    if (list.len && score_list_applies(kind)) {
+        launch_score_list(s, score, masks, n_groups, counts_rep, rep_stride, pair_rep, st, window, list, ev_start, ev_stop);
+        return;
+    }
     const bool screened = config().score_fp32_screen != 0;
     const uint32_t gpb_max = screened ? screen_gpb_max(window, thinned) : std::min<uint32_t>((uint32_t)config().score_groups_per_block, 64u);
     const uint32_t min_wgs = (uint32_t)config().score_min_workgroups;
diff --git a/misc3d_amd/csrc/m3d_cull_kernels.hpp b/misc3d_amd/csrc/m3d_cull_kernels.hpp
--- a/misc3d_amd/csrc/m3d_cull_kernels.hpp
+++ b/misc3d_amd/csrc/m3d_cull_kernels.hpp
@@ -51,6 +51,12 @@
     a.cum = reinterpret_cast<uint16_t*>(a.tiles + (size_t)kRefTileStride * a.n_tiles);
 }
 void launch_ref_hist(const RefHistArgs& a, hipStream_t st);
+constexpr uint32_t kFinalListIsKept = 0x80000000u;
+struct FinalList {
+    uint32_t* len = nullptr;
+    uint32_t* ids = nullptr;
+    const uint32_t* kept = nullptr;
+};
 void launch_plane_bound(int kind, const SortedView& s, const double* score, const unsigned long long* masks, unsigned long long* keep,
                         uint32_t n_groups, uint32_t group_begin, uint32_t group_end, uint32_t* ubsum,
                         const uint32_t* best_count, uint32_t* surv_count, const uint32_t* surv, uint32_t* tickets,
@@ -59,7 +65,8 @@
                         const unsigned long long* touched = nullptr ,
                         uint32_t touched_stride = 0,
                         const RefHistArgs* ref = nullptr ,
-                        bool ref_alone = false );
+                        bool ref_alone = false ,
+                        FinalList fin = FinalList{} );
 void launch_tile_boxes(const SortedView& s, double* boxes, hipStream_t st);
 PoisonJob make_poison_job(const SortedView& s, const double* model, double thr, uint32_t* total);
 void launch_poison_plane_inliers(const PoisonJob& job, hipStream_t st);
@@ -86,7 +93,12 @@
                        uint32_t* pair_rep ,
                        hipStream_t st, uint32_t group_begin = 0, uint32_t group_end = 0xFFFFFFFFu ,
                        hipEvent_t ev_start = nullptr, hipEvent_t ev_stop = nullptr ,
-                       bool thinned = false );
+                       bool thinned = false ,
+                       FinalList list = FinalList{} );
+bool score_list_applies(int kind);
+void launch_score_list(const SortedView& s, const double* score, const unsigned long long* masks, uint32_t n_groups,
+                       uint32_t* counts_rep, uint32_t rep_stride, uint32_t* pair_rep, hipStream_t st, uint32_t window_groups,
+                       FinalList list, hipEvent_t ev_start = nullptr, hipEvent_t ev_stop = nullptr);
 bool launch_cull_lead(int kind, const SortedView& s, const double* score, const float* cull32, unsigned long long* masks,
                       const unsigned long long* keep, uint32_t n_groups, uint32_t lead_groups, uint32_t* counts_rep,
                       uint32_t rep_stride, uint32_t* pair_rep, uint32_t* ub, uint32_t cull_end, hipStream_t st, uint32_t* ubp = nullptr);
@@ -122,7 +134,8 @@
                          uint32_t* best_count, hipStream_t st, uint32_t h_begin = 0 ,
                          uint32_t* counts_dev = nullptr ,
                          const PickFinal* pick = nullptr,
-                         const unsigned long long* keep_final = nullptr );
+                         const unsigned long long* keep_final = nullptr ,
+                         uint32_t* consumed_list_len = nullptr );
 void launch_pick_best(const uint32_t* records, uint32_t count, unsigned long long index_base, const double* params,
                       bool first_chunk, BestPick* pick, BestPickHost* pick_host, hipStream_t st,
                       uint32_t* records_host = nullptr ,
diff --git a/misc3d_amd/csrc/m3d_fit.cpp b/misc3d_amd/csrc/m3d_fit.cpp
--- a/misc3d_amd/csrc/m3d_fit.cpp
+++ b/misc3d_amd/csrc/m3d_fit.cpp
@@ -161,10 +161,10 @@
 
 constexpr size_t kBoundTicketWords = 8192;
 static int reserve_survivor_scratch(DeviceCtx* ctx, uint32_t h_pad) {
-    const size_t words = kBoundTicketWords + (size_t)h_pad + 64;
+    const size_t words = kBoundTicketWords + 2 * ((size_t)h_pad + 64);
     if ((size_t)h_pad / 64 + 2 > kBoundTicketWords) return fail(M3D_ERR_INTERNAL, "window too large for the bound's tickets");
     if (ctx->surv_list.cap < sizeof(uint32_t) * words) {
-        RESERVE(ctx->surv_list, sizeof(uint32_t) * (kBoundTicketWords + 2 * ((size_t)h_pad + 64)));
+        RESERVE(ctx->surv_list, sizeof(uint32_t) * (kBoundTicketWords + 4 * ((size_t)h_pad + 64)));
         HIPCHK(hipMemsetAsync(ctx->surv_list.p, 0, ctx->surv_list.cap, ctx->stream));
     }
     return M3D_OK;
@@ -326,6 +326,12 @@
             }
             uint32_t* const surv_count = bound_on ? bc + 6 : nullptr;
             uint32_t* const surv = bound_on ? bound_list(ctx) : nullptr;
+            FinalList fin;
+            if (bound_on && kind == M3D_PLANE && !ubp && score_list_applies(kind)) {
+                fin.len = bc + 7;
+                fin.ids = surv + ((size_t)h_pad + 64);
+                fin.kept = surv;
+            }
             unsigned long long* touched = nullptr;
             bool touched_written = false;
             if (bound_on && kind == M3D_CYLINDER && c32.out && !s.lead_fused && !(ga && g0 >= ga) && g1 - g0 >= 128u) {
@@ -363,17 +369,17 @@
             if (bound_on)
                 launch_plane_bound(kind, sv, s.score.as<double>(), masks, keep, n_groups, g_lo, g1, ubsum, bc, surv_count, surv,
                                    bound_tickets(ctx), c32.out, ctx->stream, bound_mode(kind) == 2,
-                                   touched_written && g_lo == g0 ? touched : nullptr, h_pad, ref_on ? &ref : nullptr);
+                                   touched_written && g_lo == g0 ? touched : nullptr, h_pad, ref_on ? &ref : nullptr, false, fin);
             bool phased = false;
             if (ubp)
                 phased = launch_score_phased(kind, sv, s.score.as<double>(), masks, keep, n_groups, ctx->counts_rep.as<uint32_t>(), h_pad,
                                              pair_rep, ub, ubp, bc, ctx->stream, g_lo, g1, timing ? s.k0 : nullptr, timing ? s.k1 : nullptr);
             if (!phased)
                 launch_score_mask(kind, sv, s.score.as<double>(), masks, keep, n_groups, ctx->counts_rep.as<uint32_t>(), h_pad,
-                                  pair_rep, ctx->stream, g_lo, g1, timing ? s.k0 : nullptr, timing ? s.k1 : nullptr, bound_on);
+                                  pair_rep, ctx->stream, g_lo, g1, timing ? s.k0 : nullptr, timing ? s.k1 : nullptr, bound_on, fin);
             launch_sum_replicas(ctx->counts_rep.as<uint32_t>(), h_pad, g1 * 64u, rec_host, pair_rep, h_pairs,
                                 s.valid.as<uint8_t>(), count, bc, ctx->stream, g_lo * 64u, rec_dev, pick_final ? &pfin : nullptr,
-                                phased ? keep : nullptr);
+                                phased ? keep : nullptr, fin.len);
             if (pick_final) s.poll_seq = pick_final->seq;
             s.scored = timing;
         } else {
@@ -1292,7 +1298,7 @@
     if (begin == 0) sampler->incumbent = 0;
     *ctx->h_inc.as<uint32_t>() = sampler->incumbent;
     HIPCHK(hipMemcpyAsync(ctx->best_count.p, ctx->h_inc.p, sizeof(uint32_t), hipMemcpyHostToDevice, ctx->stream));
-    HIPCHK(hipMemsetAsync(ctx->best_count.as<uint32_t>() + 6, 0, sizeof(uint32_t), ctx->stream));
+    HIPCHK(hipMemsetAsync(ctx->best_count.as<uint32_t>() + 6, 0, 2 * sizeof(uint32_t), ctx->stream));
     {
         const size_t first_own = begin + (size_t)rank * slice;
         if (rank > 0 && first_own < end) {
@@ -1481,5 +1487,57 @@
     return M3D_OK;
 }
 
-
-}
+int m3d_bench_score_list(m3d_cloud* c, double threshold, const uint32_t* samples, size_t n_hypotheses, const uint32_t* ids, size_t n_ids,
+                         uint32_t* counts_out) {
+    if (!c || !samples || !counts_out || (!ids && n_ids) || n_hypotheses == 0 || n_hypotheses > 16384 || n_ids > n_hypotheses)
+        return fail(M3D_ERR_INVALID_ARG, "invalid argument");
+    for (size_t i = 0; i < n_ids; ++i)
+        if (ids[i] >= n_hypotheses) return fail(M3D_ERR_INVALID_ARG, "list id outside the sample table");
+    DeviceCtx* ctx = c->ctx;
+    CtxLock lock(ctx);
+    HIPCHK(hipSetDevice(ctx->device));
+    if (c->work.active || c->n_tiles == 0) return fail(M3D_ERR_INVALID_ARG, "the cloud has no sorted copy of its own");
+    const CloudView v = c->view();
+    const SortedView sv = c->sorted();
+    if (!sv.tile_f32 || config().score_fp32_screen == 0) return fail(M3D_ERR_INVALID_ARG, "score_list_k needs the fp32 screen");
+    SampleSource src;
+    src.table = samples;
+    src.m = (uint32_t)minimal_sample(M3D_PLANE);
+    ChunkSlot& s = ctx->slot[0];
+    int rc = issue_chunk(ctx, s, v, sv, M3D_PLANE, threshold, 0, n_hypotheses, src, nullptr);
+    if (rc != M3D_OK) return rc;
+    const uint32_t n_groups = s.h_pad / 64;
+    RESERVE(ctx->masks, sizeof(uint64_t) * (size_t)std::max<uint32_t>(sv.n_tiles, 1) * n_groups);
+    RESERVE(ctx->counts_rep, sizeof(uint32_t) * ((size_t)kCountReplicas * s.h_pad + kPairReplicas));
+    RESERVE(ctx->small, 256);
+    RESERVE(s.counts, sizeof(uint32_t) * ((size_t)s.h_pad + 1));
+    rc = reserve_survivor_scratch(ctx, s.h_pad);
+    if (rc != M3D_OK) return rc;
+    auto* masks = ctx->masks.as<unsigned long long>();
+    uint32_t* counts_rep = ctx->counts_rep.as<uint32_t>();
+    uint32_t* ctl = ctx->small.as<uint32_t>();
+    FinalList list;
+    list.len = ctl;
+    list.ids = bound_list(ctx) + ((size_t)s.h_pad + 64);
+    const float* c32 = (!use_dense_scoring() && config().cull_fp32 != 0 && sv.radius < 1e18) ? s.cull32.as<float>() : nullptr;
+    const uint32_t len = (uint32_t)n_ids;
+    HIPCHK(hipMemsetAsync(counts_rep, 0, sizeof(uint32_t) * ((size_t)kCountReplicas * s.h_pad + kPairReplicas), ctx->stream));
+    HIPCHK(hipMemcpyAsync(ctl, &len, sizeof(len), hipMemcpyHostToDevice, ctx->stream));
+    if (n_ids) HIPCHK(hipMemcpyAsync(list.ids, ids, sizeof(uint32_t) * n_ids, hipMemcpyHostToDevice, ctx->stream));
+    launch_cull_mask(M3D_PLANE, sv, s.score.as<double>(), s.valid.as<uint8_t>(), (uint32_t)n_hypotheses, n_groups, masks, nullptr,
+                     ctx->stream, false, 0, 0xFFFFFFFFu, c32);
+    launch_score_list(sv, s.score.as<double>(), masks, n_groups, counts_rep, s.h_pad, counts_rep + (size_t)kCountReplicas * s.h_pad,
+                      ctx->stream, n_groups, list);
+    launch_sum_replicas(counts_rep, s.h_pad, s.h_pad, nullptr, nullptr, nullptr, nullptr, (uint32_t)n_hypotheses, nullptr, ctx->stream, 0,
+                        s.counts.as<uint32_t>(), nullptr, nullptr, list.len);
+    uint32_t len_after = 0;
+    HIPCHK(hipMemcpyAsync(counts_out, s.counts.p, sizeof(uint32_t) * n_hypotheses, hipMemcpyDeviceToHost, ctx->stream));
+    HIPCHK(hipMemcpyAsync(&len_after, ctl, sizeof(len_after), hipMemcpyDeviceToHost, ctx->stream));
+    HIPCHK(hipGetLastError());
+    HIPCHK(hipStreamSynchronize(ctx->stream));
+    if (len_after != 0u) return fail(M3D_ERR_INTERNAL, "the list's length word was not reset");
+    return M3D_OK;
+}
+
+
+}
```
